# Eun0/XMC-GAN

Hardware: AMD Instinct MI355X
Metric: images/sec per G+D step (higher is better)
Workload: dtype bf16; 1 GPU; 256x256 COCO-shaped synthetic batch, 256 images per GPU, one full G+D iteration (D step + G step + Adam x2), df_gan_damsm_nomagp.yml; per_gpu_batch=256, global_batch=256, image_size=256, cfg=df_gan_damsm_nomagp.yml, parallelism=dp1, hipgraph=True, losses_finite=True, workload_name=headline

## Files before the change

### include/xmc_gan_hip.h

```cpp
#ifndef XMC_GAN_HIP_H
#define XMC_GAN_HIP_H

#include <stdint.h>

#ifdef __cplusplus
extern "C" {
#endif

#define XMC_ABI_VERSION 12

enum { XMC_BF16 = 0, XMC_F32 = 1 };
enum { XMC_HALF_IS_BF16 = 0, XMC_HALF_IS_F16 = 1 };
enum { XMC_ACT_NONE = 0, XMC_ACT_LRELU = 1, XMC_ACT_TANH = 2, XMC_ACT_RELU = 3 };
enum { XMC_EINVAL = -1, XMC_EALIGN = -2, XMC_ESHAPE = -3 };

#define XMC_MAX_TAPS 16
#define XMC_MAX_CLASSES 4

typedef struct XmcConvDesc {
    const void* src;
    const void* wpk;
    void* dst;
    const float* bias;
    const void* res;
    const float* alpha_dev;
    int32_t N, SH, SW, CS;
    int32_t DH, DW, CD;
    int32_t MH, MW;
    int32_t SA, DA;
    int32_t src_shift;
    int32_t ntaps, nclass;
    int32_t CDw;
    int32_t act;
    int32_t dtype;
    int32_t out_dtype;
    int8_t dh[XMC_MAX_CLASSES][XMC_MAX_TAPS];
    int8_t dw[XMC_MAX_CLASSES][XMC_MAX_TAPS];
    int8_t wi[XMC_MAX_CLASSES][XMC_MAX_TAPS];
    int8_t dph[XMC_MAX_CLASSES];
    int8_t dpw[XMC_MAX_CLASSES];
    const void* mask;
    float res_scale;
    int32_t res_mode;
    void* dst2;
    void* dst_pool;
    int32_t round_act;
    int32_t groups;
    int32_t post_act;
    float pool_scale;
    void* sign_bits;
    float* dot;
    const void* mask_bits;
    const void* sc_img;
    const void* sc_frag;
    const float* sc_bias;
    void* splitk_ws;
    int64_t splitk_ws_bytes;
    const void* wpk_lo;
} XmcConvDesc;

int xmc_abi_version(void);
int xmc_half_format(void);
const char* xmc_last_kernel(void);
int xmc_set_fixed_order(int on);
int xmc_set_prezeroed(int on);

int64_t xmc_conv_splitk_ws_bytes(const XmcConvDesc* d);

int xmc_conv_igemm(const XmcConvDesc* d, void* stream);

int xmc_conv_wgrad(const XmcConvDesc* d , float* dwp, void* stream);
#define XMC_BIAS_REPLICAS 16
int xmc_conv_wgrad_bias(const XmcConvDesc* d, float* dwp, float* dbias, void* stream);

int xmc_pack_weight(const float* w, void* wpk, int Co, int Ci, int KH, int KW, int rows_pad, int cols_pad,
                    int transpose , int dtype, const int32_t* row_perm , void* stream);
int xmc_pack_weight_grouped(const float* w, void* wpk, int Co, int Ci, int KH, int KW, int rows_pad, int cols_pad, int transpose,
                            int dtype, const int32_t* row_perm, int groups, void* stream);
int xmc_unpack_wgrad_grouped(const float* dwp, float* gw, int Co, int Ci, int KH, int KW, int rows_pad, int cols_pad,
                             const float* scale_dev, const int32_t* row_perm, int accumulate, int groups, void* stream);
#define XMC_PACK_MULTI_MAX 48
typedef struct XmcPackJob {
    const float* w;
    void* wpk;
    const int32_t* row_perm;
    int32_t Co, Ci, KHW, rows_pad, cols_pad, transpose, dtype, groups, upconv;
    int32_t lo;
} XmcPackJob;
int xmc_pack_weight_multi(const XmcPackJob* jobs , int njobs, void* stream);
int xmc_pack_weight_upconv(const float* w, void* wpk, int Co, int Ci, int rows_pad, int cols_pad, int transpose, int dtype,
                           void* stream);
int xmc_unpack_wgrad(const float* dwp, float* gw, int Co, int Ci, int KH, int KW, int rows_pad, int cols_pad,
                     const float* scale_dev, const int32_t* row_perm, int accumulate, void* stream);
int xmc_unpack_wgrad_bias(const float* dwp, float* gw, int Co, int Ci, int KH, int KW, int rows_pad, int cols_pad,
                          const float* scale_dev, const int32_t* row_perm, int accumulate,
                          const float* gb_replicas, float* gb, int CD, void* stream);
int xmc_unpack_wgrad_bias_dot(const float* dwp, float* gw, int Co, int Ci, int KH, int KW, int rows_pad, int cols_pad,
                              const float* scale_dev, const int32_t* row_perm, int accumulate,
                              const float* gb_replicas, float* gb, int CD, const float* bias_dot, float* dot, void* stream);

int xmc_nchw_to_nhwc8(const float* src , void* dst , int N, int C, int H, int W,
                      int dtype, void* stream);
int xmc_nhwc8_to_nchw(const void* src , float* dst , int N, int C, int H, int W,
                      int dtype, void* stream);

int xmc_lrelu(const void* x, void* y, int64_t n, float slope, int dtype, void* stream);
int xmc_lrelu_mask(const void* dy, const void* ref, void* dx, int64_t n, float slope, int dtype, void* stream);
int xmc_tanh(const void* x, void* y, int64_t n, int dtype, void* stream);
int xmc_signmask_apply(const void* dy, const void* bits, void* dx, int64_t n, float slope, int dtype, void* stream);
int xmc_conv_pw1x1_masked_src(const XmcConvDesc* d, const void* src_bits, void* src_masked, float slope, void* stream);
int xmc_conv_pw1x1_split(const XmcConvDesc* d, void* stream);
int xmc_conv_ptile_bits(const XmcConvDesc* d, void* stream);
int xmc_conv_ptile_scimg(const XmcConvDesc* d, void* stream);
int xmc_conv_wgrad_bits(const XmcConvDesc* d, float* dwp, void* stream);
int xmc_gtail_bwd(const XmcConvDesc* d, const void* img, float* dwp, float* dbias, int dw_rows, int grid_cap, void* stream);
int xmc_tanh_bwd(const void* dy, const void* y, void* dx, int64_t n, int dtype, void* stream);
int xmc_axpby(const void* a, const void* b, const float* alpha_dev, void* y, int64_t n, int dtype, void* stream);
int xmc_axpby_up(const void* a, const void* b, const float* alpha_dev, void* y, int N, int H, int W, int C, int dtype, void* stream);
int xmc_axpby_up_lrelu(const void* a, const void* b, const float* alpha_dev, void* y, int N, int H, int W, int C, int dtype, void* stream);
int xmc_scale(const void* x, const float* alpha_dev, void* y, int64_t n, int dtype, void* stream);
int xmc_dot(const void* a, const void* b, float* out, int64_t n, int dtype, void* stream);
enum { XMC_GP_BIAS = 1, XMC_GP_RELU = 2, XMC_GP_MASK = 4, XMC_GP_ATOMIC = 8 };
typedef struct XmcGemmProblem {
    const float* A;
    const float* B;
    const float* bias;
    const float* mask;
    float* C;
    float* rowsum;
    int32_t M, N, K;
    int32_t sa_i, sa_r, sb_j, sb_r;
    int32_t flags;
    int32_t tile0;
    int32_t reserved;
} XmcGemmProblem;
int xmc_gemm_group(const XmcGemmProblem* problems, int nproblems, void* stream);
int xmc_embedding_gather(const int64_t* ids, const float* table, float* out, int64_t n_tokens, int dim, int64_t vocab, void* stream);
int xmc_gru_bidir(const float* xproj, const float* w_hh, const float* b_hn, const int32_t* lens, float* words, float* sent, int B, int T,
                  int H, void* stream);
int xmc_lstm_bidir(const float* xproj, const float* w_hh, const int32_t* lens, float* words, float* sent, int B, int T, int H,
                   void* stream);
int xmc_roberta_embed_ln(const int64_t* ids, const int32_t* lens, const float* word, const float* pos, const float* type0,
                         const float* gamma, const float* beta, float* out, void* out16, int B, int T, int H, int64_t vocab, int npos,
                         int pad_idx, float eps, void* stream);
int xmc_add_layernorm(const float* x, const float* bias, const float* res, const float* gamma, const float* beta, float* out, void* out16,
                      int64_t rows, int H, float eps, void* stream);
int xmc_attention_short(const float* qkv, const int32_t* lens, void* out, int B, int T, int heads, int head_dim, int out_dtype,
                        void* stream);
int xmc_bias_gelu(const float* x, const float* bias, void* out, int64_t rows, int F, int out_dtype, void* stream);
int xmc_sbert_pool(const float* hidden, const int32_t* lens, float* words, float* sent, uint8_t* mask, int B, int T, int H, int L,
                   int normalize, void* stream);
int xmc_spectral_sigma(const float* W, float* u, float* v, float* scratch, float* sig, float* w_eff, int R, int C, int training,
                       float eps, void* stream);
int xmc_spectral_bwd(const float* g, const float* W, const float* u, const float* v, const float* sig, float* dot, float* dW,
                     int R, int C, void* stream);
int xmc_scale_mask_dot(const void* dy, const void* ref, const float* alpha_dev, void* g, float* dot, int64_t n, int dtype, void* stream);
int xmc_axpby_bwd(const void* dy, const void* b, const float* alpha_dev, void* db, void* da, float* dot,
                  int N, int H, int W, int C, int up, const void* ymask , int dtype, void* stream);
int xmc_colsum(const void* x, float* out, int64_t rows, int C, int dtype, void* stream);
int xmc_avgpool2(const void* x, void* y, int N, int H, int W, int C, int dtype, void* stream);
int xmc_upsample2(const void* x, void* y, int N, int H, int W, int C, float scale, int dtype, void* stream);
int xmc_sumpool2(const void* x, void* y, int N, int H, int W, int C, float scale, int dtype, void* stream);
int xmc_global_avgpool(const void* x, void* y, int N, int HW, int C, int dtype, int out_dtype, void* stream);
int xmc_global_avgpool_bwd(const void* dy, void* dx, int N, int HW, int C, int dtype, int in_dtype, void* stream);

int xmc_affine2_lrelu_fwd(const void* x, const float* g0, const float* b0, const float* g1, const float* b1,
                          void* y, int N, int HW, int C, int dtype, void* stream);
int xmc_affine2_lrelu_bwd(const void* x, const void* dy, const float* g0, const float* b0, const float* g1,
                          const float* b1, void* dx, float* dg0, float* db0, float* dg1, float* db1,
                          int N, int HW, int C, int dtype, void* stream);

int xmc_affine2_act_fwd(const void* x, const float* g0, const float* b0, const float* g1, const float* b1,
                        void* y, int N, int HW, int C, float slope, int dtype, void* stream);
int xmc_affine2_act_bwd(const void* x, const void* dy, const float* g0, const float* b0, const float* g1,
                        const float* b1, void* dx, float* dg0, float* db0, float* dg1, float* db1,
                        int N, int HW, int C, float slope, int dtype, void* stream);
int xmc_affine2_act_bwd_acc(const void* x, const void* dy, const float* g0, const float* b0, const float* g1,
                            const float* b1, void* dx, float* dg0, float* db0, float* dg1, float* db1, const void* dx_in,
                            int N, int HW, int C, float slope, int dtype, void* stream);
int xmc_affine2_act_bwd_dot(const void* x, const void* dy, const float* g0, const float* b0, const float* g1,
                            const float* b1, void* dx, float* dg0, float* db0, float* dg1, float* db1, const void* dx_in,
                            const float* alpha_dev, float* dot, int N, int HW, int C, float slope, int dtype, void* stream);
int xmc_affine2_act_bwd_dot_pool(const void* x, const void* dy, const float* g0, const float* b0, const float* g1,
                                 const float* b1, void* dx, float* dg0, float* db0, float* dg1, float* db1, const void* dx_in,
                                 const float* alpha_dev, float* dot, void* dx_pool, int N, int H, int W, int C, float slope,
                                 int dtype, void* stream);

int xmc_groupnorm_fwd(const void* x, const float* w, const float* b, void* y, float* stats, float* ws,
                      int N, int HW, int C, int G, float eps, float slope, int dtype, void* stream);
int xmc_groupnorm_bwd(const void* x, const void* dy, const float* w, const float* b, const float* stats, void* dx,
                      float* dw, float* db, float* ws, int N, int HW, int C, int G, float slope, int dtype, void* stream);
int64_t xmc_attn_pool_ws_floats(int N, int HW);
int xmc_attn_pool_fwd(const void* key, const float* q, const void* x, float* stats, float* ctx, float* ws, int N, int HW,
                      int ncon, int pk, int px, float scale, int dtype, void* stream);
int xmc_attn_pool_bwd(const void* key, const float* q, const void* x, const float* stats, const float* ctx, const float* dctx,
                      float* dq, void* dkey, void* dx, int N, int HW, int ncon, int pk, int px, float scale, int dtype, void* stream);
int xmc_attn_pool_bwd_acc(const void* key, const float* q, const void* x, const float* stats, const float* ctx, const float* dctx,
                          float* dq, void* dkey, void* dx, const void* dx_in, int N, int HW, int ncon, int pk, int px, float scale,
                          int dtype, void* stream);

int xmc_gvec_fwd(const float* xs, const float* xg, const float* W, const float* bias, float* y, int B, int G, int O, int Is, int Ig, void* stream);
int xmc_gvec_bwd(const float* xs, const float* xg, const float* W, const float* dy, float* dxs, float* dxg, float* dW, float* dbias,
                 int B, int G, int O, int Is, int Ig, void* stream);
int xmc_reasoner_fwd(const float* x, const float* We, const float* bn_w, const float* bn_b, float* run_mean, float* run_var, int training,
                     float momentum, float eps, float* y, float* pre, float* stat, int B, void* stream);
int xmc_reasoner_bwd(const float* x, const float* We, const float* bn_w, const float* bn_b, const float* pre, const float* stat, int batch_stats,
                     const float* dy, float* dx, float* dWe, float* dbn_w, float* dbn_b, int B, void* stream);
int xmc_word_ctx_fwd(const float* st, const float* w, const unsigned char* pad, float* ctx, float* prob, int B, int T, void* stream);
int xmc_word_ctx_bwd(const float* st, const float* w, const float* prob, const float* dctx, float* dst, float* dw, int B, int T, void* stream);
int xmc_word_keys_fwd(const float* kraw, const float* gnw, const float* gnb, float eps, float* kh, float* stat, int B, int T, void* stream);
int xmc_word_keys_bwd(const float* kraw, const float* gnw, const float* gnb, const float* stat, const float* dkh, float* dkraw, float* dgnw,
                      float* dgnb, int B, int T, void* stream);
int xmc_word_pool_fwd(const void* qmap, const float* kh, const unsigned char* pad, float* ctx, int N, int HW, int ncon, int pk, int T,
                      int dtype, void* stream);
int xmc_word_pool_bwd(const void* qmap, const float* kh, const unsigned char* pad, const float* dctx, void* dq, float* dkh, int N, int HW,
                      int ncon, int pk, int T, int dtype, void* stream);

int64_t xmc_contrastive_ws_bytes(int n, int D);
int xmc_contrastive_fwd(const float* A, const float* B, const float* labels, const float* inv_num_pos,
                        int n, int D, float* loss, void* ws, void* stream);
int xmc_contrastive_bwd(const float* A, const float* B, const float* labels, const float* inv_num_pos,
                        int n, int D, const float* dloss_dev, void* ws, float* dA, float* dB, void* stream);

int xmc_cosine_scores(const float* A, const float* B, int n, int D, float* S, void* ws, void* stream);

int xmc_hinge_fwd(const void* x, int stride, float sign, float* out, int64_t n, int dtype, void* stream);
int xmc_hinge_bwd(const void* x, int stride, float sign, const float* dloss_dev, void* dx, int64_t n, int dtype,
                  void* stream);

int xmc_cast(const void* x, void* y, int64_t n, int src_dtype, int dst_dtype, void* stream);

typedef struct XmcAdamEntry {
    float* param;
    const float* grad;
    float* m;
    float* v;
    int32_t* step;
    int64_t n;
} XmcAdamEntry;
int xmc_adam_chunk_elems(void);
int xmc_adam_step(const XmcAdamEntry* table_dev, int ntensors, const int32_t* chunks_dev, int nchunks,
                  float lr, float beta1, float beta2, float eps, float grad_scale, void* stream);
enum { XMC_ADAM_CHECK = 1, XMC_ADAM_UPDATE = 2, XMC_ADAM_RESCALE = 4 };
int xmc_adam_step_scaled(const XmcAdamEntry* table_dev, int ntensors, const int32_t* chunks_dev, int nchunks,
                         float lr, float beta1, float beta2, float eps, float* scale_dev, int32_t* flags_dev,
                         int mode, float growth, float backoff, int interval, void* stream);

typedef struct XmcEmaEntry {
    float* shadow;
    const float* param;
    int64_t n;
} XmcEmaEntry;
int xmc_ema_step(const XmcEmaEntry* table_dev, int ntensors, const int32_t* chunks_dev, int nchunks, float decay, int start,
                 int32_t* num_updates_dev, const int32_t* skip_flag_dev, int bump, void* stream);
int xmc_adam_ema_step(const XmcAdamEntry* table_dev, const XmcEmaEntry* ema_table_dev, int ntensors, const int32_t* chunks_dev,
                      int nchunks, float lr, float beta1, float beta2, float eps, float grad_scale, float decay, int start,
                      int32_t* num_updates_dev, int bump, void* stream);
int xmc_adam_ema_step_scaled(const XmcAdamEntry* table_dev, const XmcEmaEntry* ema_table_dev, int ntensors,
                             const int32_t* chunks_dev, int nchunks, float lr, float beta1, float beta2, float eps,
                             float* scale_dev, int32_t* flags_dev, int mode, float growth, float backoff, int interval,
                             float decay, int start, int32_t* num_updates_dev, int bump, void* stream);

int xmc_rows_sumsq(const float* x, float* ss, int B, int64_t cols, void* stream);
int xmc_gp_finish(const float* ss, int B, float* gp, float* coef, float inv_s2, void* stream);
int xmc_rows_scale(const float* x, const float* coef, const float* g, float* y, int B, int64_t cols, void* stream);

int xmc_concept_query_fwd(const float* sent, const float* Wq, const float* gnw, const float* gnb, float* q, float* qraw,
                          int B, int E, float eps, void* stream);
// ... 81 lines not shown
```

### xmc-gan_amd/csrc/common.h

```cpp
#pragma once
#include <hip/hip_runtime.h>
#include <stdint.h>

#include "xmc_gan_hip.h"

#ifdef XMC_H16_IS_F16
typedef _Float16 xmc_h16;
#define XMC_MFMA_16x16x32 __builtin_amdgcn_mfma_f32_16x16x32_f16
#define XMC_MFMA_32x32x16 __builtin_amdgcn_mfma_f32_32x32x16_f16
#define XMC_HALF_FORMAT 1
#else
typedef __bf16 xmc_h16;
#define XMC_MFMA_16x16x32 __builtin_amdgcn_mfma_f32_16x16x32_bf16
#define XMC_MFMA_32x32x16 __builtin_amdgcn_mfma_f32_32x32x16_bf16
#define XMC_HALF_FORMAT 0
#endif
typedef __attribute__((ext_vector_type(8))) xmc_h16 bf16x8;
typedef __attribute__((ext_vector_type(4))) xmc_h16 bf16x4;
typedef __attribute__((ext_vector_type(4))) float f32x4;
typedef __attribute__((__vector_size__(4 * sizeof(short)))) short xmc_s16x4;
typedef __attribute__((ext_vector_type(4))) uint32_t u32x4;
typedef __attribute__((ext_vector_type(2))) uint32_t u32x2;

#define XMC_LRELU 0.2f

static inline int xmc_esz(int dtype) { return dtype == XMC_BF16 ? 2 : 4; }

void xmc_note_kernel(const char* fmt, ...);
void xmc_note_generic_epi(const char* kernel, int mask);
bool xmc_debug_off(const char* token);
bool xmc_fixed_order();
hipError_t xmc_zero_acc(void* p, size_t bytes, hipStream_t st);

#define XMC_LAUNCH_CHECK()                                     \
    do {                                                       \
        hipError_t e__ = hipGetLastError();                    \
        if (e__ != hipSuccess) return -(1000 + (int)e__);      \
    } while (0)

#define XMC_MAX_DYN_LDS (160 * 1024 - 1024)
#define XMC_ALLOW_BIG_LDS(kernel)                                                                                              \
    do {                                                                                                                       \
        static bool once__ = false;                                                                                            \
        if (!once__) {                                                                                                         \
            (void)hipFuncSetAttribute(reinterpret_cast<const void*>(&kernel), hipFuncAttributeMaxDynamicSharedMemorySize,      \
                                      XMC_MAX_DYN_LDS);                                                                        \
            (void)hipGetLastError();                                                                                           \
            once__ = true;                                                                                                     \
        }                                                                                                                      \
    } while (0)

__device__ __forceinline__ bf16x4 xmc_ds_read_tr16(const void* p) {
    return __builtin_bit_cast(bf16x4, __builtin_amdgcn_ds_read_tr16_b64_v4i16((__attribute__((address_space(3))) xmc_s16x4*)(p)));
}

__device__ __forceinline__ float xmc_pin_f32(float v) {
    asm("" : "+v"(v));
    return v;
}
__device__ __forceinline__ float lrelu_f(float v) { return v > 0.f ? v : XMC_LRELU * v; }
__device__ __forceinline__ float tanh_fast(float v) {
    const float e = __builtin_amdgcn_exp2f(v * 2.8853900817779268f);
    return 1.f - 2.f * __builtin_amdgcn_rcpf(e + 1.f);
}
__device__ __forceinline__ float lrelu_slope(float ref) { return ref > 0.f ? 1.f : XMC_LRELU; }
__device__ __forceinline__ float tanh_bwd_f(float dy, float y) { return xmc_pin_f32(dy * (1.f - y * y)); }
__device__ __forceinline__ u32x4 xmc_apply_sign_bits(u32x4 v, unsigned b) {
    bf16x8 h = __builtin_bit_cast(bf16x8, v);
#pragma unroll
    for (int k = 0; k < 8; ++k) {
        const float f = (float)h[k];
        h[k] = (xmc_h16)(((b >> k) & 1u) ? f : XMC_LRELU * f);
    }
    return __builtin_bit_cast(u32x4, h);
}

template <int DT> struct Vec8;
template <> struct Vec8<XMC_BF16> {
    static constexpr int BYTES = 16;
    __device__ static __forceinline__ void load(const void* p, size_t idx8, float (&v)[8]) {
        bf16x8 t = reinterpret_cast<const bf16x8*>(p)[idx8];
#pragma unroll
        for (int i = 0; i < 8; ++i) v[i] = (float)t[i];
    }
    __device__ static __forceinline__ void store(void* p, size_t idx8, const float (&v)[8]) {
        bf16x8 t;
#pragma unroll
        for (int i = 0; i < 8; ++i) t[i] = (xmc_h16)v[i];
        reinterpret_cast<bf16x8*>(p)[idx8] = t;
    }
};
template <> struct Vec8<XMC_F32> {
    static constexpr int BYTES = 32;
    __device__ static __forceinline__ void load(const void* p, size_t idx8, float (&v)[8]) {
        const f32x4* q = reinterpret_cast<const f32x4*>(p) + idx8 * 2;
        f32x4 a = q[0], b = q[1];
#pragma unroll
        for (int i = 0; i < 4; ++i) { v[i] = a[i]; v[4 + i] = b[i]; }
    }
    __device__ static __forceinline__ void store(void* p, size_t idx8, const float (&v)[8]) {
        f32x4* q = reinterpret_cast<f32x4*>(p) + idx8 * 2;
        f32x4 a, b;
#pragma unroll
        for (int i = 0; i < 4; ++i) { a[i] = v[i]; b[i] = v[4 + i]; }
        q[0] = a; q[1] = b;
    }
};

struct XcdWalk { int first, step, end; };
__device__ __forceinline__ XcdWalk xmc_xcd_walk(int ntiles) {
    const int G = (int)gridDim.x, b = (int)blockIdx.x;
#ifdef XMC_XCD_HELPER_OFF
    return XcdWalk{b, G, ntiles};
#endif
    if ((G & 7) != 0 || G < 16) return XcdWalk{b, G, ntiles};
    const int T8 = (ntiles + 7) >> 3, base = (b & 7) * T8;
    return XcdWalk{base + (b >> 3), G >> 3, base + T8 < ntiles ? base + T8 : ntiles};
}
static inline int xmc_ab_grid(int g) {
    static const bool off = xmc_debug_off("no_xcd_map");
    return (off && g >= 16 && (g & 7) == 0) ? g - 1 : g;
}

__device__ __forceinline__ float xmc_xor1(float v) {
    return __builtin_bit_cast(float, __builtin_amdgcn_mov_dpp(__builtin_bit_cast(int, v), 0xB1, 0xF, 0xF, true));
}
__device__ __forceinline__ float xmc_xor2(float v) {
    return __builtin_bit_cast(float, __builtin_amdgcn_mov_dpp(__builtin_bit_cast(int, v), 0x4E, 0xF, 0xF, true));
}
__device__ __forceinline__ float wave_sum(float v) {
#pragma unroll
    for (int o = 32; o > 0; o >>= 1) v += __shfl_xor(v, o, 64);
    return v;
}
__device__ __forceinline__ float wave_max(float v) {
#pragma unroll
    for (int o = 32; o > 0; o >>= 1) v = fmaxf(v, __shfl_xor(v, o, 64));
    return v;
}

template <int ODT>
__device__ __forceinline__ void epilogue_tail(const XmcConvDesc& d, size_t idx8, size_t ridx8, float (&v)[8], float alpha, float* dacc = nullptr) {
    if (d.sign_bits) {
        unsigned b = 0;
#pragma unroll
        for (int k = 0; k < 8; ++k) b |= (v[k] > 0.f ? 1u : 0u) << k;
        reinterpret_cast<unsigned char*>(d.sign_bits)[idx8] = (unsigned char)b;
    }
    if (d.dst2) Vec8<ODT>::store(d.dst2, idx8, v);
    if (ODT == XMC_BF16 && (d.dst2 || d.round_act)) {
#pragma unroll
        for (int k = 0; k < 8; ++k) v[k] = (float)(xmc_h16)v[k];
    }
    float mk[8];
    if (d.mask) {
        Vec8<ODT>::load(d.mask, idx8, mk);
        if (d.dot && dacc) {
#pragma unroll
            for (int k = 0; k < 8; ++k) *dacc += v[k] * mk[k];
        }
    }
    if (d.alpha_dev) {
#pragma unroll
        for (int k = 0; k < 8; ++k) v[k] *= alpha;
    }
    if (d.mask) {
#pragma unroll
        for (int k = 0; k < 8; ++k) v[k] *= lrelu_slope(mk[k]);
    }
    if (d.res) {
        const float rs = d.res_scale == 0.f ? 1.f : d.res_scale;
        float rr[8];
        Vec8<ODT>::load(d.res, ridx8, rr);
#pragma unroll
        for (int k = 0; k < 8; ++k) v[k] += rs * rr[k];
    }
    if (d.post_act == XMC_ACT_LRELU) {
#pragma unroll
        for (int k = 0; k < 8; ++k) v[k] = lrelu_f(v[k]);
    }
    Vec8<ODT>::store(d.dst, idx8, v);
}

constexpr int kEpiBias = 1, kEpiLrelu = 2, kEpiRound = 4, kEpiDst2 = 8, kEpiAlpha = 16, kEpiMask = 32, kEpiRes = 64, kEpiPost = 128, kEpiPool = 256,
              kEpiSign = 512, kEpiDot = 1024, kEpiScImg = 2048;
constexpr int kEpiGSum = kEpiBias | kEpiRound | kEpiAlpha | kEpiRes;
constexpr int kEpiDKeep = kEpiLrelu | kEpiDst2 | kEpiAlpha | kEpiRes | kEpiPool;
constexpr int kEpiDFwd = kEpiLrelu | kEpiRound | kEpiAlpha | kEpiRes | kEpiPool;
constexpr int kEpiDLast = kEpiLrelu | kEpiDst2 | kEpiAlpha | kEpiRes;
constexpr int kEpiDLin = kEpiDst2 | kEpiAlpha | kEpiMask | kEpiRes;
constexpr int kEpiDKeepS = kEpiLrelu | kEpiRound | kEpiSign | kEpiAlpha | kEpiRes | kEpiPool;
constexpr int kEpiDLastS = kEpiLrelu | kEpiRound | kEpiSign | kEpiAlpha | kEpiRes;
constexpr int kEpiDgDot = kEpiMask | kEpiAlpha | kEpiDot;
static inline int xmc_epi_mask(const XmcConvDesc& d) {
    if ((d.act != XMC_ACT_NONE && d.act != XMC_ACT_LRELU) || d.out_dtype != XMC_BF16) return -1;
    return (d.bias ? kEpiBias : 0) | (d.act == XMC_ACT_LRELU ? kEpiLrelu : 0) | ((d.round_act && !d.dst2) ? kEpiRound : 0) | (d.dst2 ? kEpiDst2 : 0) |
           (d.alpha_dev ? kEpiAlpha : 0) | (d.mask ? kEpiMask : 0) | (d.res ? kEpiRes : 0) | (d.post_act == XMC_ACT_LRELU ? kEpiPost : 0) |
           (d.dst_pool ? kEpiPool : 0) | (d.sign_bits ? kEpiSign : 0) | (d.dot ? kEpiDot : 0) | (d.sc_img ? kEpiScImg : 0);
}

__device__ __forceinline__ size_t res_index8(const XmcConvDesc& d, size_t idx8, int n, int y, int x, int a, int b, int ch8) {
    if (d.res_mode == 0) return idx8;
    if (d.res_mode == 1) return ((size_t)(n * d.MH + a) * d.MW + b) * (d.CD >> 3) + ch8;
    return ((size_t)(n * (d.DH >> 1) + (y >> 1)) * (d.DW >> 1) + (x >> 1)) * (d.CD >> 3) + ch8;
}
```

### xmc-gan_amd/csrc/conv_thin.hip

```cpp
#include "common.h"
#include <stdlib.h>

namespace {

struct ThinCfg {
    int tiles_y, tiles_x, PW, PH, dh0, dw0;
};

template <int BN>
__global__ __launch_bounds__(256) void thin_in_kernel(const XmcConvDesc d, const ThinCfg t, int ntiles) {
    constexpr int TH = 8, TW = 32, TN = BN / 16, UPL = BN / 32, KS = 3;
    __shared__ __attribute__((aligned(16))) unsigned char patch[(TH + 4) * (TW + 4) * 16];
    const int tid = threadIdx.x, lane = tid & 63, wm = tid >> 6;
    const int fr = lane & 15, fc = lane >> 4;
    const int PW = t.PW, PH = t.PH, dh0 = t.dh0, dw0 = t.dw0;
    const u32x4* __restrict__ src16 = reinterpret_cast<const u32x4*>(d.src);
    const u32x4* __restrict__ w16 = reinterpret_cast<const u32x4*>(d.wpk);

    u32x4 wf[KS][TN];
    int toff[KS];
#pragma unroll
    for (int ks = 0; ks < KS; ++ks) {
        const int tap = ks * 4 + fc;
        const bool live = tap < d.ntaps;
// ... 393 lines not shown
#pragma unroll
            for (int u = 0; u < TN / 2; ++u) {
                if (u * 32 + fc * 8 >= d.CD) continue;
                bf16x8 o;
#pragma unroll
                for (int q = 0; q < 4; ++q) {
                    const float x0 = acc[2 * u][q] + bias8[u][q], x1 = acc[2 * u + 1][q] + bias8[u][4 + q];
                    o[q] = (xmc_h16)fmaxf(x0, x0 * slope);
                    o[4 + q] = (xmc_h16)fmaxf(x1, x1 * slope);
                }
                dst8[pix * cd8 + u * 4 + fc] = o;
            }
        }
    }
}

template <int KS, int TN>
int launch_pw(const XmcConvDesc& d, int ngroups, hipStream_t st, const unsigned char* sbits, void* smasked, float mslope) {
    int nb = (ngroups + 4 * 4 - 1) / (4 * 4);
    if (nb > 256 * 8) nb = 256 * 8;
    if (d.wpk_lo) {
        if constexpr ((KS == 2 && TN == 8) || (KS == 4 && TN == 4) || (KS == 2 && TN == 2)) {
            if (smasked) return 1;
            hipLaunchKernelGGL((pw1x1_kernel<KS, TN, false, true>), dim3(nb), dim3(256), 0, st, d, ngroups, nullptr, nullptr, 0.f);
            xmc_note_kernel("pw1x1_kernel<%d, %d, false, true>", KS, TN);
            XMC_LAUNCH_CHECK();
            return 0;
        } else {
            return 1;
        }
    }
    if (smasked) hipLaunchKernelGGL((pw1x1_kernel<KS, TN, true>), dim3(nb), dim3(256), 0, st, d, ngroups, sbits, (u32x4*)smasked, mslope);
    else hipLaunchKernelGGL((pw1x1_kernel<KS, TN, false>), dim3(nb), dim3(256), 0, st, d, ngroups, nullptr, nullptr, 0.f);
    xmc_note_kernel(smasked ? "pw1x1_kernel<%d, %d, true>" : "pw1x1_kernel<%d, %d>", KS, TN);
    XMC_LAUNCH_CHECK();
    return 0;
}

template <int KS, bool MASKED = false, bool SPLIT = false>
__global__ __launch_bounds__(512) void pw1x1w_kernel(const XmcConvDesc d, int ngroups, int ncols, const unsigned char* __restrict__ sbits,
                                                     u32x4* __restrict__ smasked, float mslope) {
    extern __shared__ __attribute__((aligned(16))) unsigned char wlds[];
    constexpr int RSTR = KS * 64 * (SPLIT ? 2 : 1) + 16;
    const int tid = threadIdx.x, lane = tid & 63, fr = lane & 15, fc = lane >> 4;
    const int cs_units = d.CS >> 3, cd8 = d.CD >> 3;
    const int c0 = blockIdx.y * ncols;
    const u32x4* __restrict__ src16 = reinterpret_cast<const u32x4*>(d.src);
    const u32x4* __restrict__ w16 = reinterpret_cast<const u32x4*>(d.wpk);
    bf16x8* __restrict__ dst8 = reinterpret_cast<bf16x8*>(d.dst);
    for (int id = tid; id < ncols * KS * 4; id += 512) {
        const int row = id / (KS * 4), ch = id - row * (KS * 4);
        const int j = row >> 4, r = row & 15;
        const int lrow = (j >> 1) * 32 + (r >> 2) * 8 + (j & 1) * 4 + (r & 3);
        *reinterpret_cast<u32x4*>(wlds + row * RSTR + ch * 16) = w16[((size_t)d.wi[0][0] * d.CDw + c0 + lrow) * cs_units + ch];
        if (SPLIT) *reinterpret_cast<u32x4*>(wlds + row * RSTR + KS * 64 + ch * 16) =
                reinterpret_cast<const u32x4*>(d.wpk_lo)[((size_t)d.wi[0][0] * d.CDw + c0 + lrow) * cs_units + ch];
    }
    __syncthreads();
    const float slope = d.act == XMC_ACT_LRELU ? XMC_LRELU : 1.f;
    const int wave_g = blockIdx.x * 8 + (tid >> 6), nwaves = gridDim.x * 8;
    constexpr int UNR = 4;
    const int nu = ncols >> 5;
    for (int g0 = wave_g * UNR; g0 < ngroups; g0 += nwaves * UNR) {
        u32x4 pf[UNR][KS];
#pragma unroll
        for (int r = 0; r < UNR; ++r) {
            const int g = g0 + r < ngroups ? g0 + r : ngroups - 1;
#pragma unroll
            for (int ks = 0; ks < KS; ++ks) pf[r][ks] = src16[(size_t)(g * 16 + fr) * cs_units + ks * 4 + fc];
        }
        if (MASKED && blockIdx.y == 0) {
#pragma unroll
            for (int r = 0; r < UNR; ++r) {
                if (g0 + r >= ngroups) break;
#pragma unroll
                for (int ks = 0; ks < KS; ++ks) {
                    const size_t idx = (size_t)((g0 + r) * 16 + fr) * cs_units + ks * 4 + fc;
                    smasked[idx] = mask_unit(pf[r][ks], sbits[idx], mslope);
                }
            }
        }
        for (int u = 0; u < nu; ++u) {
            f32x4 acc[UNR][2];
#pragma unroll
            for (int r = 0; r < UNR; ++r) acc[r][0] = acc[r][1] = f32x4{0.f, 0.f, 0.f, 0.f};
            const unsigned char* const wr = wlds + (u * 32 + fr) * RSTR + fc * 16;
#pragma unroll
            for (int ks = 0; ks < KS; ++ks) {
                const bf16x8 wa = *reinterpret_cast<const bf16x8*>(wr + ks * 64), wb = *reinterpret_cast<const bf16x8*>(wr + 16 * RSTR + ks * 64);
                if (SPLIT) {
                    const bf16x8 la = *reinterpret_cast<const bf16x8*>(wr + KS * 64 + ks * 64), lb = *reinterpret_cast<const bf16x8*>(wr + 16 * RSTR + KS * 64 + ks * 64);
#pragma unroll
                    for (int r = 0; r < UNR; ++r) {
                        acc[r][0] = XMC_MFMA_16x16x32(la, __builtin_bit_cast(bf16x8, pf[r][ks]), acc[r][0], 0, 0, 0);
                        acc[r][1] = XMC_MFMA_16x16x32(lb, __builtin_bit_cast(bf16x8, pf[r][ks]), acc[r][1], 0, 0, 0);
                    }
                }
#pragma unroll
                for (int r = 0; r < UNR; ++r) {
                    acc[r][0] = XMC_MFMA_16x16x32(wa, __builtin_bit_cast(bf16x8, pf[r][ks]), acc[r][0], 0, 0, 0);
                    acc[r][1] = XMC_MFMA_16x16x32(wb, __builtin_bit_cast(bf16x8, pf[r][ks]), acc[r][1], 0, 0, 0);
                }
            }
            const int ch = c0 + u * 32 + fc * 8;
            if (ch >= d.CD) continue;
            float b8[8];
#pragma unroll
            for (int c = 0; c < 8; ++c) b8[c] = d.bias ? d.bias[ch + c] : 0.f;
#pragma unroll
            for (int r = 0; r < UNR; ++r) {
                if (g0 + r >= ngroups) break;
                bf16x8 o;
#pragma unroll
                for (int q = 0; q < 4; ++q) {
                    const float x0 = acc[r][0][q] + b8[q], x1 = acc[r][1][q] + b8[4 + q];
                    o[q] = (xmc_h16)fmaxf(x0, x0 * slope);
                    o[4 + q] = (xmc_h16)fmaxf(x1, x1 * slope);
                }
                dst8[((size_t)(g0 + r) * 16 + fr) * cd8 + (ch >> 3)] = o;
            }
        }
    }
}

template <int KS>
int launch_pww(const XmcConvDesc& d, int ngroups, hipStream_t st, const unsigned char* sbits, void* smasked, float mslope) {
    const bool split = d.wpk_lo != nullptr;
    if (split && smasked) return 1;
    const int RSTR = KS * 64 * (split ? 2 : 1) + 16;
    int ny = 1;
    while ((size_t)(d.CDw / ny) * RSTR > XMC_MAX_DYN_LDS || d.CDw % ny != 0 || (d.CDw / ny) % 32 != 0) {
        if (++ny > d.CDw / 32) return 1;
    }
    const int ncols = d.CDw / ny;
    const size_t lds = (size_t)ncols * RSTR;
    int nb = (ngroups + 8 * 4 - 1) / (8 * 4);
    if (nb > 256 / ny) nb = 256 / ny;
    if (nb < 1) nb = 1;
    if (split) {
        XMC_ALLOW_BIG_LDS((pw1x1w_kernel<KS, false, true>));
        hipLaunchKernelGGL((pw1x1w_kernel<KS, false, true>), dim3(nb, ny), dim3(512), lds, st, d, ngroups, ncols, nullptr, nullptr, 0.f);
        xmc_note_kernel("pw1x1w_kernel<%d, false, true>", KS);
        XMC_LAUNCH_CHECK();
        return 0;
    }
    if (smasked) {
        XMC_ALLOW_BIG_LDS((pw1x1w_kernel<KS, true>));
        hipLaunchKernelGGL((pw1x1w_kernel<KS, true>), dim3(nb, ny), dim3(512), lds, st, d, ngroups, ncols, sbits, (u32x4*)smasked, mslope);
    } else {
        XMC_ALLOW_BIG_LDS((pw1x1w_kernel<KS, false>));
        hipLaunchKernelGGL((pw1x1w_kernel<KS, false>), dim3(nb, ny), dim3(512), lds, st, d, ngroups, ncols, nullptr, nullptr, 0.f);
    }
    xmc_note_kernel(smasked ? "pw1x1w_kernel<%d, true>" : "pw1x1w_kernel<%d>", KS);
    XMC_LAUNCH_CHECK();
    return 0;
}

constexpr int TO_H = 8, TO_W = 16, TO_PH = TO_H + 2, TO_PW = TO_W + 2;
template <int KC>
__global__ __launch_bounds__(256, 2) void thin_out_kernel(const XmcConvDesc d, int tiles_x, int tiles_y, int ntiles) {
    constexpr int NKS = 9 * KC, CSU = 4 * KC, PSTR = CSU * 16 + 16;
    constexpr int NUN = TO_PH * TO_PW * CSU, MAXU = (NUN + 255) / 256;
    __shared__ __attribute__((aligned(16))) unsigned char smem[TO_PH * TO_PW * PSTR];
    const int tid = threadIdx.x, lane = tid & 63, wave = tid >> 6;
    const int col = lane & 15, kb = lane >> 4;
    const u32x4* __restrict__ src = reinterpret_cast<const u32x4*>(d.src);
    const u32x4* __restrict__ wpk = reinterpret_cast<const u32x4*>(d.wpk);
    bf16x8 wa[NKS];
    int loff[9];
#pragma unroll
    for (int t = 0; t < 9; ++t) {
        loff[t] = ((d.dh[0][t] + 1) * TO_PW + d.dw[0][t] + 1 + col) * PSTR + kb * 16;
#pragma unroll
        for (int c = 0; c < KC; ++c)
            wa[t * KC + c] = __builtin_bit_cast(bf16x8, wpk[((size_t)d.wi[0][t] * d.CDw + col) * CSU + c * 4 + kb]);
    }
    float bias4[4] = {0.f, 0.f, 0.f, 0.f};
    if (d.bias && kb < 2) {
#pragma unroll
        for (int i = 0; i < 4; ++i) bias4[i] = d.bias[kb * 4 + i];
    }
    u32x4 pv[MAXU];
    auto prefetch = [&](int tile) {
        const int n = tile / (tiles_y * tiles_x), tr = tile - n * (tiles_y * tiles_x);
        const int y0 = (tr / tiles_x) * TO_H - 1, x0 = (tr % tiles_x) * TO_W - 1;
#pragma unroll
        for (int it = 0; it < MAXU; ++it) {
            const int id = tid + it * 256;
            const int pp = id / CSU, ch = id - pp * CSU;
            const int py = pp / TO_PW, px = pp - py * TO_PW;
            const int sy = y0 + py, sx = x0 + px;
            const bool ok = id < NUN && (unsigned)sy < (unsigned)d.SH && (unsigned)sx < (unsigned)d.SW;
            const u32x4 z = {0, 0, 0, 0};
            pv[it] = ok ? src[(((size_t)n * d.SH + sy) * d.SW + sx) * CSU + ch] : z;
        }
    };
    const XcdWalk xw = xmc_xcd_walk(ntiles);
    int tile = xw.first;
    if (tile < xw.end) prefetch(tile);
    for (; tile < xw.end; tile += xw.step) {
        __syncthreads();
#pragma unroll
        for (int it = 0; it < MAXU; ++it) {
            const int id = tid + it * 256;
            const int pp = id / CSU, ch = id - pp * CSU;
            if (id < NUN) *reinterpret_cast<u32x4*>(smem + pp * PSTR + ch * 16) = pv[it];
        }
        __syncthreads();
        if (tile + xw.step < xw.end) prefetch(tile + xw.step);
        const int n = tile / (tiles_y * tiles_x), tr = tile - n * (tiles_y * tiles_x);
        const int y0 = (tr / tiles_x) * TO_H, x0 = (tr % tiles_x) * TO_W;
#pragma unroll
        for (int rr = 0; rr < 2; ++rr) {
            const int r = wave * 2 + rr;
            f32x4 acc = {0.f, 0.f, 0.f, 0.f};
#pragma unroll
            for (int t = 0; t < 9; ++t)
#pragma unroll
                for (int c = 0; c < KC; ++c) {
                    const bf16x8 b = *reinterpret_cast<const bf16x8*>(smem + r * TO_PW * PSTR + loff[t] + c * 64);
                    acc = XMC_MFMA_16x16x32(wa[t * KC + c], b, acc, 0, 0, 0);
                }
            if (kb < 2) {
                bf16x4 o;
#pragma unroll
                for (int i = 0; i < 4; ++i) {
                    float v = acc[i] + bias4[i];
                    if (d.act == XMC_ACT_TANH) v = tanh_fast(v);
                    else if (d.act == XMC_ACT_LRELU) v = lrelu_f(v);
                    o[i] = (xmc_h16)v;
                }
                const size_t p = ((size_t)n * d.DH + y0 + r) * d.DW + x0 + col;
                *reinterpret_cast<bf16x4*>(reinterpret_cast<xmc_h16*>(d.dst) + p * 8 + kb * 4) = o;
            }
        }
    }
}

}

int xmc_conv_thin_out_try(const XmcConvDesc* d, void* stream) {
    static const bool off = xmc_debug_off("no_thin_out");
    if (off) return 1;
    if (d->dtype != XMC_BF16 || d->out_dtype != XMC_BF16 || d->CD != 8 || (d->CS != 32 && d->CS != 64) || d->CDw < 16) return 1;
    if (d->SA != 1 || d->DA != 1 || d->src_shift != 0 || d->nclass != 1 || d->ntaps != 9 || d->groups > 1) return 1;
    if (d->res || d->mask || d->alpha_dev || d->dst2 || d->dst_pool || d->post_act || d->sign_bits || d->dot) return 1;
    if (d->act != XMC_ACT_NONE && d->act != XMC_ACT_TANH && d->act != XMC_ACT_LRELU) return 1;
    if (d->MH % TO_H != 0 || d->MW % TO_W != 0 || d->SH != d->MH || d->SW != d->MW || d->DH != d->MH || d->DW != d->MW) return 1;
    if (d->dph[0] != 0 || d->dpw[0] != 0) return 1;
    for (int k = 0; k < 9; ++k)
        if (d->dh[0][k] < -1 || d->dh[0][k] > 1 || d->dw[0][k] < -1 || d->dw[0][k] > 1) return 1;
    const int tx = d->MW / TO_W, ty = d->MH / TO_H, ntiles = d->N * tx * ty;
    const int grid = ntiles < 256 * 8 ? ntiles : 256 * 8;
    hipStream_t st = reinterpret_cast<hipStream_t>(stream);
    if (d->CS == 32) hipLaunchKernelGGL((thin_out_kernel<1>), dim3(xmc_ab_grid(grid)), dim3(256), 0, st, *d, tx, ty, ntiles);
    else hipLaunchKernelGGL((thin_out_kernel<2>), dim3(xmc_ab_grid(grid)), dim3(256), 0, st, *d, tx, ty, ntiles);
    xmc_note_kernel("thin_out_kernel<%d>", d->CS / 32);
    XMC_LAUNCH_CHECK();
    return 0;
}

int xmc_conv_thin_try(const XmcConvDesc* d, void* stream) {
    static const bool off = xmc_debug_off("no_thin");
    if (off) return 1;
    if (d->dtype != XMC_BF16 || d->out_dtype != XMC_BF16 || d->CS != 8) return 1;
    if (d->SA != 1 || d->DA != 1 || d->src_shift != 0 || d->nclass != 1 || d->ntaps > 12) return 1;
    if (d->CDw != 32 && d->CDw != 64) return 1;
    if (d->res || d->alpha_dev || d->dst2 || d->post_act || d->sign_bits || d->dot || (d->act != XMC_ACT_NONE && d->act != XMC_ACT_LRELU)) return 1;
    if (d->MH % 8 != 0 || d->MW % 32 != 0 || d->SH != d->MH || d->SW != d->MW || d->DH != d->MH || d->DW != d->MW) return 1;
    if (d->dph[0] != 0 || d->dpw[0] != 0) return 1;
    int hmin = 127, hmax = -128, wmin = 127, wmax = -128;
    for (int k = 0; k < d->ntaps; ++k) {
        const int h = d->dh[0][k], w = d->dw[0][k];
        hmin = h < hmin ? h : hmin; hmax = h > hmax ? h : hmax;
        wmin = w < wmin ? w : wmin; wmax = w > wmax ? w : wmax;
    }
    if (hmax - hmin > 4 || wmax - wmin > 4 || hmin > 0 || wmin > 0 || hmax < 0 || wmax < 0) return 1;
    ThinCfg t;
    t.tiles_y = d->MH / 8; t.tiles_x = d->MW / 32;
    t.PH = 8 + (hmax - hmin); t.PW = 32 + (wmax - wmin);
    t.dh0 = hmin; t.dw0 = wmin;
    if (t.PH * t.PW > 512) return 1;
    const int ntiles = d->N * t.tiles_y * t.tiles_x;
    int gx = 256 * 5;
    if (gx > ntiles) gx = ntiles;
    hipStream_t st = reinterpret_cast<hipStream_t>(stream);
    if (d->CDw == 32) {
        hipLaunchKernelGGL((thin_in_kernel<32>), dim3(xmc_ab_grid(gx)), dim3(256), 0, st, *d, t, ntiles);
    } else {
        hipLaunchKernelGGL((thin_in_kernel<64>), dim3(xmc_ab_grid(gx)), dim3(256), 0, st, *d, t, ntiles);
    }
    xmc_note_kernel("thin_in_kernel<%d>", d->CDw);
    XMC_LAUNCH_CHECK();
    return 0;
}

extern "C" int xmc_gtail_bwd(const XmcConvDesc* d, const void* img, float* dwp, float* dbias, int dw_rows, int grid_cap, void* stream) {
    if (!d || !d->src || !d->wpk || !d->dst || !d->mask || !img) return XMC_EINVAL;
    if (d->N < 1 || d->MH < 1 || d->MW < 1 || d->ntaps < 1 || d->ntaps > XMC_MAX_TAPS) return XMC_ESHAPE;
    if (dwp && (dw_rows < 4 || dw_rows % 4 != 0)) return XMC_ESHAPE;
    if (d->mask_bits || d->sc_img || d->wpk_lo) return XMC_EINVAL;
    static const bool off = xmc_debug_off("no_gtail_fused");
    if (off) return 1;
    if (d->dtype != XMC_BF16 || d->out_dtype != XMC_BF16 || d->CS != 8 || d->CD != 32 || d->CDw != 32) return 1;
    if (d->SA != 1 || d->DA != 1 || d->src_shift != 0 || d->nclass != 1 || d->ntaps != 9 || d->groups > 1) return 1;
    if (d->bias || d->res || d->alpha_dev || d->dst2 || d->post_act || d->sign_bits || d->dot || d->act != XMC_ACT_NONE) return 1;
    if (d->MH % 8 != 0 || d->MW % 2 != 0 || d->SH != d->MH || d->SW != d->MW || d->DH != d->MH || d->DW != d->MW) return 1;
    if (d->dph[0] != 0 || d->dpw[0] != 0) return 1;
    for (int t = 0; t < 9; ++t)
        if (d->dh[0][t] != 1 - t / 3 || d->dw[0][t] != 1 - t % 3 || d->wi[0][t] != t) return 1;
    const int tiles_y = d->MH / 8, tiles_x = (d->MW + 31) / 32;
    if ((int64_t)d->N * d->MH * d->MW * 4 >= (1ll << 31) || (int64_t)d->N * tiles_y * tiles_x >= (1ll << 30)) return 1;
    const int ntiles = d->N * tiles_y * tiles_x;
    int gx = 256 * (dwp ? 3 : 5);
    if (grid_cap > 0 && gx > grid_cap) gx = grid_cap;
    if (gx > ntiles) gx = ntiles;
    hipStream_t st = reinterpret_cast<hipStream_t>(stream);
    const u32x4* img16 = reinterpret_cast<const u32x4*>(img);
    if (dwp) hipLaunchKernelGGL((gtail_bwd_kernel<true>), dim3(xmc_ab_grid(gx)), dim3(256), 0, st, *d, img16, dwp, dbias, dw_rows, tiles_y, tiles_x, ntiles);
    else hipLaunchKernelGGL((gtail_bwd_kernel<false>), dim3(xmc_ab_grid(gx)), dim3(256), 0, st, *d, img16, nullptr, nullptr, 0, tiles_y, tiles_x, ntiles);
    xmc_note_kernel("gtail_bwd_kernel<%d>", dwp ? 1 : 0);
    XMC_LAUNCH_CHECK();
    return 0;
}

static int pw1x1_go(const XmcConvDesc* d, void* stream, const unsigned char* sbits, void* smasked, float mslope) {
    static const bool off = xmc_debug_off("no_pw1x1");
    if (off) return 1;
    if (d->dtype != XMC_BF16 || d->out_dtype != XMC_BF16) return 1;
    if (d->ntaps != 1 || d->nclass != 1 || d->SA != 1 || d->DA != 1 || d->src_shift != 0) return 1;
    if (d->dh[0][0] != 0 || d->dw[0][0] != 0 || d->dph[0] != 0 || d->dpw[0] != 0) return 1;
    if (d->SH != d->MH || d->SW != d->MW || d->DH != d->MH || d->DW != d->MW) return 1;
    if (d->post_act || d->sign_bits || d->dot) return 1;
    if (d->res || d->mask || d->alpha_dev || d->dst2 || (d->act != XMC_ACT_NONE && d->act != XMC_ACT_LRELU)) return 1;
    if (d->CS % 32 != 0 || d->CDw % 32 != 0 || d->CD % 8 != 0) return 1;
    const int64_t M = (int64_t)d->N * d->MH * d->MW;
    if (M % 16 != 0 || M / 16 >= (1ll << 31) || M < 16 * 1024) return 1;
    const int ngroups = (int)(M / 16);
    hipStream_t st = reinterpret_cast<hipStream_t>(stream);
    const int ks = d->CS / 32, tn = d->CDw / 16;
    static const bool no_w = xmc_debug_off("no_pw1x1_lds");
    if (!no_w && (ks == 4 || ks == 8) && ks * tn > 16 && d->CDw >= 128 && M >= 32 * 1024)
        return ks == 4 ? launch_pww<4>(*d, ngroups, st, sbits, smasked, mslope) : launch_pww<8>(*d, ngroups, st, sbits, smasked, mslope);
    if (d->CS > 128 || d->CDw > 128) return 1;
    if (ks * tn > 16 || ks == 3) return 1;
#define PW_CASE(K, T) if (ks == K && tn == T) return launch_pw<K, T>(*d, ngroups, st, sbits, smasked, mslope);
    PW_CASE(1, 2) PW_CASE(1, 4) PW_CASE(1, 8) PW_CASE(2, 2) PW_CASE(2, 4) PW_CASE(2, 8) PW_CASE(4, 2) PW_CASE(4, 4)
#undef PW_CASE
    return 1;
}

int xmc_conv_pw1x1_try(const XmcConvDesc* d, void* stream) { return d->wpk_lo ? 1 : pw1x1_go(d, stream, nullptr, nullptr, 0.f); }

extern "C" int xmc_conv_pw1x1_split(const XmcConvDesc* d, void* stream) {
    if (!d || !d->src || !d->wpk || !d->wpk_lo || !d->dst) return XMC_EINVAL;
    if (d->ntaps != 1 || d->CS % 8 != 0 || d->CD % 8 != 0 || d->CDw % 32 != 0 || d->CDw < d->CD || d->N < 1 || d->MH < 1 || d->MW < 1) return XMC_ESHAPE;
    if (d->mask_bits || d->sc_img) return XMC_EINVAL;
    static const bool off = xmc_debug_off("no_pw1x1_split");
    if (off) return 1;
    return pw1x1_go(d, stream, nullptr, nullptr, 0.f);
}

extern "C" int xmc_conv_pw1x1_masked_src(const XmcConvDesc* d, const void* src_bits, void* src_masked, float slope, void* stream) {
    if (!d || !d->src || !d->wpk || !d->dst || !src_bits || !src_masked) return XMC_EINVAL;
    if (d->ntaps != 1 || d->CS % 8 != 0 || d->CD % 8 != 0 || d->CDw % 32 != 0 || d->CDw < d->CD || d->N < 1 || d->MH < 1 || d->MW < 1) return XMC_ESHAPE;
    static const bool off = xmc_debug_off("no_pw1x1_masked_src");
    if (off) return 1;
    return pw1x1_go(d, stream, static_cast<const unsigned char*>(src_bits), src_masked, slope);
}
```

### xmc-gan_amd/csrc/pointwise.hip

```cpp
#include "common.h"
#include <stdlib.h>
#include <string.h>
#include <cstdarg>
#include <cstdio>

namespace {

constexpr int NT = 256;
inline int nblocks(int64_t items, int per_block = NT, int cap = 256 * 16) {
    int64_t b = (items + per_block - 1) / per_block;
    if (b < 1) b = 1;
    return (int)(b > cap ? cap : b);
}

constexpr int UN = 4;
constexpr int STREAM_BLOCKS = 1024;
inline int sblocks(int64_t n8) { return nblocks((n8 + UN - 1) / UN, NT, STREAM_BLOCKS); }

template <int DT, class F>
__global__ void map1_kernel(const void* x, void* y, int64_t n8, F f) {
    for (int64_t base = (int64_t)blockIdx.x * (NT * UN); base < n8; base += (int64_t)gridDim.x * (NT * UN)) {
        float v[UN][8];
#pragma unroll
        for (int j = 0; j < UN; ++j) {
// ... 175 lines not shown
    }
    __shared__ float red[NT * 8];
#pragma unroll
    for (int k = 0; k < 8; ++k) red[threadIdx.x * 8 + k] = s[k];
    __syncthreads();
    if (threadIdx.x < c8_here) {
        float t[8] = {0, 0, 0, 0, 0, 0, 0, 0};
        for (int gg = 0; gg < groups; ++gg)
#pragma unroll
            for (int k = 0; k < 8; ++k) t[k] += red[(gg * c8_here + threadIdx.x) * 8 + k];
#pragma unroll
        for (int k = 0; k < 8; ++k) atomicAdd(&out[(c8_base + threadIdx.x) * 8 + k], t[k]);
    }
}

template <int DT>
__global__ void pool2_kernel(const void* x, void* y, int N, int H, int W, int C8, float scale) {
    const int OH = H / 2, OW = W / 2;
    const int64_t total = (int64_t)N * OH * OW * C8;
    for (int64_t i = blockIdx.x * (int64_t)blockDim.x + threadIdx.x; i < total; i += (int64_t)gridDim.x * blockDim.x) {
        int cc = (int)(i % C8);
        int64_t p = i / C8;
        int ow = (int)(p % OW); p /= OW;
        int oh = (int)(p % OH);
        int n = (int)(p / OH);
        float acc[8] = {0, 0, 0, 0, 0, 0, 0, 0}, v[8];
#pragma unroll
        for (int dy = 0; dy < 2; ++dy)
#pragma unroll
            for (int dx = 0; dx < 2; ++dx) {
                Vec8<DT>::load(x, (((int64_t)n * H + 2 * oh + dy) * W + 2 * ow + dx) * C8 + cc, v);
#pragma unroll
                for (int k = 0; k < 8; ++k) acc[k] += v[k];
            }
#pragma unroll
        for (int k = 0; k < 8; ++k) acc[k] *= scale;
        Vec8<DT>::store(y, i, acc);
    }
}
template <int DT>
__global__ void up2_kernel(const void* x, void* y, int N, int H, int W, int C8, float scale) {
    const int OH = H * 2, OW = W * 2;
    const int64_t total = (int64_t)N * OH * OW * C8;
    for (int64_t i = blockIdx.x * (int64_t)blockDim.x + threadIdx.x; i < total; i += (int64_t)gridDim.x * blockDim.x) {
        int cc = (int)(i % C8);
        int64_t p = i / C8;
        int ow = (int)(p % OW); p /= OW;
        int oh = (int)(p % OH);
        int n = (int)(p / OH);
        float v[8];
        Vec8<DT>::load(x, (((int64_t)n * H + (oh >> 1)) * W + (ow >> 1)) * C8 + cc, v);
#pragma unroll
        for (int k = 0; k < 8; ++k) v[k] *= scale;
        Vec8<DT>::store(y, i, v);
    }
}
template <int DT, int OD>
__global__ void gap_kernel(const void* x, void* y, int N, int HW, int C8) {
    const int64_t total = (int64_t)N * C8;
    for (int64_t i = blockIdx.x * (int64_t)blockDim.x + threadIdx.x; i < total; i += (int64_t)gridDim.x * blockDim.x) {
        int cc = (int)(i % C8);
        int n = (int)(i / C8);
        float acc[8] = {0, 0, 0, 0, 0, 0, 0, 0}, v[8];
        for (int p = 0; p < HW; ++p) {
            Vec8<DT>::load(x, ((int64_t)n * HW + p) * C8 + cc, v);
#pragma unroll
            for (int k = 0; k < 8; ++k) acc[k] += v[k];
        }
        const float inv = 1.f / HW;
#pragma unroll
        for (int k = 0; k < 8; ++k) acc[k] *= inv;
        Vec8<OD>::store(y, i, acc);
    }
}
template <int DT>
__global__ void gap_big_kernel(const void* x, float* y, int HW, int C8, int pix_per_block) {
    const int n = blockIdx.y, groups = NT / C8;
    const int cc = threadIdx.x % C8, g = threadIdx.x / C8;
    float acc[8] = {0, 0, 0, 0, 0, 0, 0, 0}, v[8];
    const int p_end = min(HW, (int)(blockIdx.x + 1) * pix_per_block);
    if (g < groups)
        for (int p = blockIdx.x * pix_per_block + g; p < p_end; p += groups) {
            Vec8<DT>::load(x, ((size_t)n * HW + p) * C8 + cc, v);
#pragma unroll
            for (int k = 0; k < 8; ++k) acc[k] += v[k];
        }
    __shared__ float red[NT * 8];
#pragma unroll
    for (int k = 0; k < 8; ++k) red[threadIdx.x * 8 + k] = acc[k];
    __syncthreads();
    if (threadIdx.x < C8) {
        const float inv = 1.f / HW;
        float t[8] = {0, 0, 0, 0, 0, 0, 0, 0};
        for (int gg = 0; gg < groups; ++gg)
#pragma unroll
            for (int k = 0; k < 8; ++k) t[k] += red[(gg * C8 + threadIdx.x) * 8 + k];
#pragma unroll
        for (int k = 0; k < 8; ++k) atomicAdd(&y[((size_t)n * C8 + threadIdx.x) * 8 + k], t[k] * inv);
    }
}
template <int DT, int ID>
__global__ void gap_bwd_kernel(const void* dy, void* dx, int N, int HW, int C8) {
    const int64_t total = (int64_t)N * HW * C8;
    const float inv = 1.f / HW;
    for (int64_t i = blockIdx.x * (int64_t)blockDim.x + threadIdx.x; i < total; i += (int64_t)gridDim.x * blockDim.x) {
        int cc = (int)(i % C8);
        int n = (int)(i / ((int64_t)HW * C8));
        float v[8];
        Vec8<ID>::load(dy, (int64_t)n * C8 + cc, v);
#pragma unroll
        for (int k = 0; k < 8; ++k) v[k] *= inv;
        Vec8<DT>::store(dx, i, v);
    }
}

template <int DT>
__global__ void nchw_to_nhwc8_kernel(const float* src, void* dst, int N, int C, int HW) {
    const int64_t total = (int64_t)N * HW;
    for (int64_t i = blockIdx.x * (int64_t)blockDim.x + threadIdx.x; i < total; i += (int64_t)gridDim.x * blockDim.x) {
        int64_t n = i / HW, p = i - n * HW;
        float v[8] = {0, 0, 0, 0, 0, 0, 0, 0};
        for (int c = 0; c < C; ++c) v[c] = src[(n * C + c) * HW + p];
        Vec8<DT>::store(dst, i, v);
    }
}
template <int DT>
__global__ void nhwc8_to_nchw_kernel(const void* src, float* dst, int N, int C, int HW) {
    const int64_t total = (int64_t)N * HW;
    for (int64_t i = blockIdx.x * (int64_t)blockDim.x + threadIdx.x; i < total; i += (int64_t)gridDim.x * blockDim.x) {
        int64_t n = i / HW, p = i - n * HW;
        float v[8];
        Vec8<DT>::load(src, i, v);
        for (int c = 0; c < C; ++c) dst[(n * C + c) * HW + p] = v[c];
    }
}

template <int DT>
__global__ void affine2_fwd_kernel(const void* x, const float* g0, const float* b0, const float* g1, const float* b1,
                                   void* y, int HW, int C8, int pix_per_block, float slope) {
    const int n = blockIdx.y, groups = NT / C8;
    const int cc = threadIdx.x % C8, g = threadIdx.x / C8;
    if (g >= groups) return;
    float G0[8], B0[8], G1[8], B1[8];
    const size_t pb = ((size_t)n * C8 + cc) * 8;
    const bool two = g1 != nullptr;
#pragma unroll
    for (int k = 0; k < 8; ++k) { G0[k] = g0[pb + k]; B0[k] = b0[pb + k]; G1[k] = two ? g1[pb + k] : 1.f; B1[k] = two ? b1[pb + k] : 0.f; }
    const int p_end = min(HW, (int)(blockIdx.x + 1) * pix_per_block);
    for (int p = blockIdx.x * pix_per_block + g; p < p_end; p += groups) {
        float v[8];
        const size_t idx = ((size_t)n * HW + p) * C8 + cc;
        Vec8<DT>::load(x, idx, v);
#pragma unroll
        for (int k = 0; k < 8; ++k) {
            float u = v[k] * G0[k] + B0[k];
            u = u > 0.f ? u : slope * u;
            const float t = u * G1[k] + B1[k];
            v[k] = two ? (t > 0.f ? t : slope * t) : u;
        }
        Vec8<DT>::store(y, idx, v);
    }
}
template <int DT, bool POOL>
__global__ __launch_bounds__(NT, 2) void affine2_bwd_kernel(
                                   const void* x, const void* dy, const float* g0, const float* b0, const float* g1,
                                   const float* b1, void* dx, float* dg0, float* db0, float* dg1, float* db1,
                                   int HW, int C8, int pix_per_block, float slope, const void* dx_in,
                                   const float* alpha_dev, float* dot, void* dx_pool, int Wq) {
    const float al = alpha_dev ? *alpha_dev : 1.f;
    float dacc = 0.f;
    const int n = blockIdx.y, groups = NT / C8;
    const int cc = threadIdx.x % C8, g = threadIdx.x / C8;
    float G0[8], B0[8], G1[8], B1[8];
    float sg0[8], sb0[8], sg1[8], sb1[8];
    const size_t pb = ((size_t)n * C8 + cc) * 8;
    const bool two = g1 != nullptr;
#pragma unroll
    for (int k = 0; k < 8; ++k) {
        G0[k] = g0[pb + k]; B0[k] = b0[pb + k]; G1[k] = two ? g1[pb + k] : 1.f; B1[k] = two ? b1[pb + k] : 0.f;
        sg0[k] = sb0[k] = sg1[k] = sb1[k] = 0.f;
    }
    auto pixel = [&](size_t idx, float (&xv)[8], const float (&dv)[8], const float (&o)[8], float* acc8) {
#pragma unroll
        for (int k = 0; k < 8; ++k) {
            float u = xv[k] * G0[k] + B0[k];
            float a1 = u > 0.f ? u : slope * u;
            float v = a1 * G1[k] + B1[k];
            if (dot) {
                const float y2 = two ? (v > 0.f ? v : slope * v) : a1;
                dacc += dv[k] * (DT == XMC_BF16 ? (float)(xmc_h16)y2 : y2);
            }
            const float dvk = dv[k] * al;
            float dvv = two ? dvk * (v > 0.f ? 1.f : slope) : dvk;
            sg1[k] += dvv * a1; sb1[k] += dvv;
            float du = dvv * G1[k] * (u > 0.f ? 1.f : slope);
            sg0[k] += du * xv[k]; sb0[k] += du;
            xv[k] = du * G0[k];
        }
        if (dx_in) {
#pragma unroll
            for (int k = 0; k < 8; ++k) xv[k] += o[k];
        }
        Vec8<DT>::store(dx, idx, xv);
        if (POOL) {
#pragma unroll
            for (int k = 0; k < 8; ++k) acc8[k] += DT == XMC_BF16 ? (float)(xmc_h16)xv[k] : xv[k];
        }
    };
    const int p_end = min(HW, (int)(blockIdx.x + 1) * pix_per_block);
    if (g < groups)
        for (int p = blockIdx.x * pix_per_block + g; p < p_end; p += POOL ? groups : 2 * groups) {
            if (!POOL) {
                float xv[8], dv[8], o[8], xw[8], dw[8], ow[8];
                const size_t idx = ((size_t)n * HW + p) * C8 + cc;
                const bool second = p + groups < p_end;
                const size_t idx2 = second ? idx + (size_t)groups * C8 : idx;
                Vec8<DT>::load(x, idx, xv);
                Vec8<DT>::load(x, idx2, xw);
                Vec8<DT>::load(dy, idx, dv);
                Vec8<DT>::load(dy, idx2, dw);
                if (dx_in) { Vec8<DT>::load(dx_in, idx, o); Vec8<DT>::load(dx_in, idx2, ow); }
                pixel(idx, xv, dv, o, nullptr);
                if (second) pixel(idx2, xw, dw, ow, nullptr);
            } else {
                const int W = 2 * Wq;
                const int qy = p / W, col = p - qy * W;
                const size_t i0 = (((size_t)n * (HW / W) * 2 + 2 * qy) * W + col) * C8 + cc, i1 = i0 + (size_t)W * C8;
                float x0[8], d0[8], o0[8], x1[8], d1[8], o1[8];
                Vec8<DT>::load(x, i0, x0); Vec8<DT>::load(x, i1, x1);
                Vec8<DT>::load(dy, i0, d0); Vec8<DT>::load(dy, i1, d1);
                if (dx_in) { Vec8<DT>::load(dx_in, i0, o0); Vec8<DT>::load(dx_in, i1, o1); }
                float acc8[8] = {0, 0, 0, 0, 0, 0, 0, 0};
                pixel(i0, x0, d0, o0, acc8);
                pixel(i1, x1, d1, o1, acc8);
#pragma unroll
                for (int k = 0; k < 8; ++k) acc8[k] += __shfl_xor(acc8[k], C8, 64);
                if ((col & 1) == 0) Vec8<DT>::store(dx_pool, (((size_t)n * (HW / W) + qy) * Wq + (col >> 1)) * C8 + cc, acc8);
            }
        }
    if (dot) {
        dacc = wave_sum(dacc);
        if ((threadIdx.x & 63) == 0) atomicAdd(dot, dacc);
    }
    __shared__ float red[NT * 8];
    float* outs[4] = {dg0, db0, dg1, db1};
    float* sums[4] = {sg0, sb0, sg1, sb1};
#pragma unroll
    for (int q = 0; q < 4; ++q) {
        if (!two && q >= 2) break;
        __syncthreads();
#pragma unroll
        for (int k = 0; k < 8; ++k) red[threadIdx.x * 8 + k] = sums[q][k];
        __syncthreads();
        if (threadIdx.x < C8) {
            float t[8] = {0, 0, 0, 0, 0, 0, 0, 0};
            for (int gg = 0; gg < groups; ++gg)
#pragma unroll
                for (int k = 0; k < 8; ++k) t[k] += red[(gg * C8 + threadIdx.x) * 8 + k];
#pragma unroll
            for (int k = 0; k < 8; ++k) atomicAdd(&outs[q][((size_t)n * C8 + threadIdx.x) * 8 + k], t[k]);
        }
    }
}

template <int DT>
__global__ void hinge_fwd_kernel(const void* x, int stride, float sign, float* out, int64_t n) {
    float s = 0.f;
    for (int64_t i = threadIdx.x; i < n; i += blockDim.x) {
        float v = DT == XMC_BF16 ? (float)reinterpret_cast<const xmc_h16*>(x)[i * stride] : reinterpret_cast<const float*>(x)[i * stride];
        s += fmaxf(1.f + sign * v, 0.f);
    }
    s = wave_sum(s);
    __shared__ float part[NT / 64];
    if ((threadIdx.x & 63) == 0) part[threadIdx.x >> 6] = s;
    __syncthreads();
    if (threadIdx.x == 0) {
        float t = 0.f;
        for (int w = 0; w < NT / 64; ++w) t += part[w];
        *out = t / (float)n;
    }
}
template <int DT>
__global__ void hinge_bwd_kernel(const void* x, int stride, float sign, const float* dloss, void* dx, int64_t n) {
    const float gscale = (*dloss) * sign / (float)n;
    for (int64_t i = blockIdx.x * (int64_t)blockDim.x + threadIdx.x; i < n; i += (int64_t)gridDim.x * blockDim.x) {
        float v = DT == XMC_BF16 ? (float)reinterpret_cast<const xmc_h16*>(x)[i * stride] : reinterpret_cast<const float*>(x)[i * stride];
        float gval = (1.f + sign * v) > 0.f ? gscale : 0.f;
        if (DT == XMC_BF16) reinterpret_cast<xmc_h16*>(dx)[i * stride] = (xmc_h16)gval;
        else reinterpret_cast<float*>(dx)[i * stride] = gval;
    }
}

__device__ __forceinline__ float pack_value(const float* __restrict__ w, int Co, int Ci, int KHW, int rows_pad, int cols_pad,
                                            int transpose, const int32_t* __restrict__ row_perm, int groups, int64_t i) {
    const int cog = Co / groups, cig = Ci / groups;
    int c = (int)(i % cols_pad);
    int64_t q = i / cols_pad;
    int r = (int)(q % rows_pad);
    int t = (int)(q / rows_pad);
    int co = transpose ? c : r, ci = transpose ? r : c;
    float v = 0.f;
    if (co < Co && ci < Ci) {
        int sco = row_perm ? row_perm[co] : co;
        if (groups == 1) v = w[((int64_t)sco * Ci + ci) * KHW + t];
        else if (sco / cog == ci / cig) v = w[((int64_t)sco * cig + ci % cig) * KHW + t];
    }
    return v;
}
__device__ __forceinline__ float pack_upconv_value(const float* __restrict__ w, int Co, int Ci, int rows_pad, int cols_pad,
                                                   int transpose, int64_t idx) {
    int c = (int)(idx % cols_pad);
    int64_t q = idx / cols_pad;
    int r = (int)(q % rows_pad);
    int sl = (int)(q / rows_pad);
    int cls = sl >> 2, t = sl & 3;
    int i = cls >> 1, j = cls & 1, th = t >> 1, tw = t & 1;
    int co = transpose ? c : r, ci = transpose ? r : c;
    float v = 0.f;
    if (co < Co && ci < Ci) {
        int kh0 = (i == 0) ? (th == 0 ? 0 : 1) : (th == 0 ? 0 : 2), kh1 = (i == 0) ? (th == 0 ? 0 : 2) : (th == 0 ? 1 : 2);
        int kw0 = (j == 0) ? (tw == 0 ? 0 : 1) : (tw == 0 ? 0 : 2), kw1 = (j == 0) ? (tw == 0 ? 0 : 2) : (tw == 0 ? 1 : 2);
        const float* wp = w + ((int64_t)co * Ci + ci) * 9;
        for (int kh = kh0; kh <= kh1; ++kh)
            for (int kw = kw0; kw <= kw1; ++kw) v += wp[kh * 3 + kw];
    }
    return v;
}
template <int DT>
__global__ void pack_weight_kernel(const float* w, void* wpk, int Co, int Ci, int KHW, int rows_pad, int cols_pad,
                                   int transpose, const int32_t* row_perm, int groups) {
    const int64_t total = (int64_t)KHW * rows_pad * cols_pad;
    for (int64_t i = blockIdx.x * (int64_t)blockDim.x + threadIdx.x; i < total; i += (int64_t)gridDim.x * blockDim.x) {
        const float v = pack_value(w, Co, Ci, KHW, rows_pad, cols_pad, transpose, row_perm, groups, i);
        if (DT == XMC_BF16) reinterpret_cast<xmc_h16*>(wpk)[i] = (xmc_h16)v;
        else reinterpret_cast<float*>(wpk)[i] = v;
    }
}
template <int DT>
__global__ void pack_upconv_kernel(const float* w, void* wpk, int Co, int Ci, int rows_pad, int cols_pad, int transpose) {
    const int64_t total = (int64_t)16 * rows_pad * cols_pad;
    for (int64_t idx = blockIdx.x * (int64_t)blockDim.x + threadIdx.x; idx < total; idx += (int64_t)gridDim.x * blockDim.x) {
        const float v = pack_upconv_value(w, Co, Ci, rows_pad, cols_pad, transpose, idx);
        if (DT == XMC_BF16) reinterpret_cast<xmc_h16*>(wpk)[idx] = (xmc_h16)v;
        else reinterpret_cast<float*>(wpk)[idx] = v;
    }
}
constexpr int PM_CHUNK = 2048;
struct PackJobs { XmcPackJob j[XMC_PACK_MULTI_MAX]; int32_t first[XMC_PACK_MULTI_MAX + 1]; int32_t njobs; };
template <int DT>
__device__ __forceinline__ void pack_store(void* p, int64_t i, float v, bool lo = false) {
    if (DT == XMC_BF16) reinterpret_cast<xmc_h16*>(p)[i] = lo ? (xmc_h16)(v - (float)(xmc_h16)v) : (xmc_h16)v;
    else reinterpret_cast<float*>(p)[i] = v;
}
template <int DT>
__device__ __forceinline__ void pack_position(const XmcPackJob& job, int pos) {
// ... 622 lines not shown
```

### xmc-gan_amd/lib.py

```python
import ctypes as C
import os

HERE = os.path.dirname(os.path.abspath(__file__))
LIB_PATH = os.environ.get("XMC_LIB_PATH", os.path.join(HERE, "libxmc_gan_hip.so"))
LIB_PATH_F16 = os.environ.get("XMC_LIB_PATH_F16", os.path.join(HERE, "libxmc_gan_hip_f16.so"))
ABI_VERSION = 12

BF16, F32 = 0, 1
H16 = BF16
ACT_NONE, ACT_LRELU, ACT_TANH, ACT_RELU = 0, 1, 2, 3
MAX_TAPS, MAX_CLASSES = 16, 4
POOL_MAX, POOL_AVG_VALID, POOL_AVG_PAD = 0, 1, 2
DIFFAUG_PARTS = 64

vp, i32, i64, f32 = C.c_void_p, C.c_int32, C.c_int64, C.c_float


class ConvDesc(C.Structure):
    _fields_ = [("src", vp), ("wpk", vp), ("dst", vp), ("bias", vp), ("res", vp), ("alpha_dev", vp),
                ("N", i32), ("SH", i32), ("SW", i32), ("CS", i32),
                ("DH", i32), ("DW", i32), ("CD", i32),
                ("MH", i32), ("MW", i32), ("SA", i32), ("DA", i32), ("src_shift", i32),
                ("ntaps", i32), ("nclass", i32), ("CDw", i32), ("act", i32), ("dtype", i32), ("out_dtype", i32),
                ("dh", (C.c_int8 * MAX_TAPS) * MAX_CLASSES), ("dw", (C.c_int8 * MAX_TAPS) * MAX_CLASSES),
                ("wi", (C.c_int8 * MAX_TAPS) * MAX_CLASSES),
                ("dph", C.c_int8 * MAX_CLASSES), ("dpw", C.c_int8 * MAX_CLASSES),
                ("mask", vp), ("res_scale", f32), ("res_mode", i32), ("dst2", vp), ("dst_pool", vp), ("round_act", i32), ("groups", i32),
                ("post_act", i32), ("pool_scale", f32), ("sign_bits", vp), ("dot", vp), ("mask_bits", vp), ("sc_img", vp), ("sc_frag", vp), ("sc_bias", vp),
                ("splitk_ws", vp), ("splitk_ws_bytes", C.c_int64), ("wpk_lo", vp)]


GEMM_PROBLEM = [("A", "u8"), ("B", "u8"), ("bias", "u8"), ("mask", "u8"), ("C", "u8"), ("rowsum", "u8"),
                ("M", "i4"), ("N", "i4"), ("K", "i4"), ("sa_i", "i4"), ("sa_r", "i4"), ("sb_j", "i4"), ("sb_r", "i4"),
                ("flags", "i4"), ("tile0", "i4"), ("reserved", "i4")]
GP_BIAS, GP_RELU, GP_MASK, GP_ATOMIC = 1, 2, 4, 8


class PackJob(C.Structure):
    _fields_ = [("w", vp), ("wpk", vp), ("row_perm", vp), ("Co", i32), ("Ci", i32), ("KHW", i32), ("rows_pad", i32),
                ("cols_pad", i32), ("transpose", i32), ("dtype", i32), ("groups", i32), ("upconv", i32), ("lo", i32)]


class AdamEntry(C.Structure):
    _fields_ = [("param", vp), ("grad", vp), ("m", vp), ("v", vp), ("step", vp), ("n", i64)]


class EmaEntry(C.Structure):
    _fields_ = [("shadow", vp), ("param", vp), ("n", i64)]


_SIGS = {
    "xmc_abi_version": [],
    "xmc_half_format": [],
    "xmc_last_kernel": [],
    "xmc_set_fixed_order": [i32],
    "xmc_set_prezeroed": [i32],
    "xmc_conv_splitk_ws_bytes": [vp],
    "xmc_conv_igemm": [C.POINTER(ConvDesc), vp],
    "xmc_conv_wgrad": [C.POINTER(ConvDesc), vp, vp],
    "xmc_conv_wgrad_bias": [C.POINTER(ConvDesc), vp, vp, vp],
    "xmc_pack_weight": [vp, vp, i32, i32, i32, i32, i32, i32, i32, i32, vp, vp],
    "xmc_pack_weight_grouped": [vp, vp, i32, i32, i32, i32, i32, i32, i32, i32, vp, i32, vp],
    "xmc_pack_weight_upconv": [vp, vp, i32, i32, i32, i32, i32, i32, vp],
    "xmc_pack_weight_multi": [C.POINTER(PackJob), i32, vp],
    "xmc_axpby_up": [vp, vp, vp, vp, i32, i32, i32, i32, i32, vp],
    "xmc_unpack_wgrad": [vp, vp, i32, i32, i32, i32, i32, i32, vp, vp, i32, vp],
    "xmc_unpack_wgrad_grouped": [vp, vp, i32, i32, i32, i32, i32, i32, vp, vp, i32, i32, vp],
    "xmc_unpack_wgrad_bias": [vp, vp, i32, i32, i32, i32, i32, i32, vp, vp, i32, vp, vp, i32, vp],
    "xmc_unpack_wgrad_bias_dot": [vp, vp, i32, i32, i32, i32, i32, i32, vp, vp, i32, vp, vp, i32, vp, vp, vp],
    "xmc_nchw_to_nhwc8": [vp, vp, i32, i32, i32, i32, i32, vp],
    "xmc_nhwc8_to_nchw": [vp, vp, i32, i32, i32, i32, i32, vp],
    "xmc_lrelu": [vp, vp, i64, f32, i32, vp],
    "xmc_lrelu_mask": [vp, vp, vp, i64, f32, i32, vp],
    "xmc_tanh": [vp, vp, i64, i32, vp],
    "xmc_signmask_apply": [vp, vp, vp, i64, f32, i32, vp],
    "xmc_conv_pw1x1_masked_src": [C.POINTER(ConvDesc), vp, vp, f32, vp],
    "xmc_conv_pw1x1_split": [C.POINTER(ConvDesc), vp],
    "xmc_conv_ptile_bits": [C.POINTER(ConvDesc), vp],
    "xmc_conv_ptile_scimg": [C.POINTER(ConvDesc), vp],
    "xmc_conv_wgrad_bits": [C.POINTER(ConvDesc), vp, vp],
    "xmc_gtail_bwd": [C.POINTER(ConvDesc), vp, vp, vp, i32, i32, vp],
    "xmc_tanh_bwd": [vp, vp, vp, i64, i32, vp],
    "xmc_axpby": [vp, vp, vp, vp, i64, i32, vp],
    "xmc_scale_mask_dot": [vp, vp, vp, vp, vp, i64, i32, vp],
    "xmc_axpby_bwd": [vp, vp, vp, vp, vp, vp, i32, i32, i32, i32, i32, vp, i32, vp],
    "xmc_axpby_up_lrelu": [vp, vp, vp, vp, i32, i32, i32, i32, i32, vp],
    "xmc_scale": [vp, vp, vp, i64, i32, vp],
    "xmc_dot": [vp, vp, vp, i64, i32, vp],
    "xmc_gemm_group": [vp, i32, vp],
    "xmc_embedding_gather": [vp, vp, vp, i64, i32, i64, vp],
    "xmc_lstm_bidir": [vp, vp, vp, vp, vp, i32, i32, i32, vp],
    "xmc_gru_bidir": [vp, vp, vp, vp, vp, vp, i32, i32, i32, vp],
    "xmc_roberta_embed_ln": [vp, vp, vp, vp, vp, vp, vp, vp, vp, i32, i32, i32, i64, i32, i32, f32, vp],
    "xmc_add_layernorm": [vp, vp, vp, vp, vp, vp, vp, i64, i32, f32, vp],
    "xmc_attention_short": [vp, vp, vp, i32, i32, i32, i32, i32, vp],
    "xmc_bias_gelu": [vp, vp, vp, i64, i32, i32, vp],
    "xmc_sbert_pool": [vp, vp, vp, vp, vp, i32, i32, i32, i32, i32, vp],
    "xmc_spectral_sigma": [vp, vp, vp, vp, vp, vp, i32, i32, i32, f32, vp],
    "xmc_spectral_bwd": [vp, vp, vp, vp, vp, vp, vp, i32, i32, vp],
    "xmc_colsum": [vp, vp, i64, i32, i32, vp],
    "xmc_avgpool2": [vp, vp, i32, i32, i32, i32, i32, vp],
    "xmc_upsample2": [vp, vp, i32, i32, i32, i32, f32, i32, vp],
    "xmc_sumpool2": [vp, vp, i32, i32, i32, i32, f32, i32, vp],
    "xmc_global_avgpool": [vp, vp, i32, i32, i32, i32, i32, vp],
    "xmc_global_avgpool_bwd": [vp, vp, i32, i32, i32, i32, i32, vp],
    "xmc_affine2_act_fwd": [vp, vp, vp, vp, vp, vp, i32, i32, i32, f32, i32, vp],
    "xmc_affine2_act_bwd": [vp, vp, vp, vp, vp, vp, vp, vp, vp, vp, vp, i32, i32, i32, f32, i32, vp],
    "xmc_affine2_act_bwd_acc": [vp, vp, vp, vp, vp, vp, vp, vp, vp, vp, vp, vp, i32, i32, i32, f32, i32, vp],
    "xmc_affine2_act_bwd_dot": [vp, vp, vp, vp, vp, vp, vp, vp, vp, vp, vp, vp, vp, vp, i32, i32, i32, f32, i32, vp],
    "xmc_affine2_act_bwd_dot_pool": [vp, vp, vp, vp, vp, vp, vp, vp, vp, vp, vp, vp, vp, vp, vp, i32, i32, i32, i32, f32, i32, vp],
    "xmc_affine2_lrelu_fwd": [vp, vp, vp, vp, vp, vp, i32, i32, i32, i32, vp],
    "xmc_affine2_lrelu_bwd": [vp, vp, vp, vp, vp, vp, vp, vp, vp, vp, vp, i32, i32, i32, i32, vp],
    "xmc_groupnorm_fwd": [vp, vp, vp, vp, vp, vp, i32, i32, i32, i32, f32, f32, i32, vp],
    "xmc_groupnorm_bwd": [vp, vp, vp, vp, vp, vp, vp, vp, vp, i32, i32, i32, i32, f32, i32, vp],
    "xmc_attn_pool_ws_floats": [i32, i32],
    "xmc_attn_pool_fwd": [vp, vp, vp, vp, vp, vp, i32, i32, i32, i32, i32, f32, i32, vp],
    "xmc_attn_pool_bwd": [vp, vp, vp, vp, vp, vp, vp, vp, vp, i32, i32, i32, i32, i32, f32, i32, vp],
    "xmc_attn_pool_bwd_acc": [vp, vp, vp, vp, vp, vp, vp, vp, vp, vp, i32, i32, i32, i32, i32, f32, i32, vp],
    "xmc_word_pool_fwd": [vp, vp, vp, vp, i32, i32, i32, i32, i32, i32, vp],
    "xmc_word_pool_bwd": [vp, vp, vp, vp, vp, vp, i32, i32, i32, i32, i32, i32, vp],
    "xmc_gvec_fwd": [vp, vp, vp, vp, vp, i32, i32, i32, i32, i32, vp],
    "xmc_gvec_bwd": [vp, vp, vp, vp, vp, vp, vp, vp, i32, i32, i32, i32, i32, vp],
    "xmc_reasoner_fwd": [vp, vp, vp, vp, vp, vp, i32, f32, f32, vp, vp, vp, i32, vp],
    "xmc_reasoner_bwd": [vp, vp, vp, vp, vp, vp, i32, vp, vp, vp, vp, vp, i32, vp],
    "xmc_word_ctx_fwd": [vp, vp, vp, vp, vp, i32, i32, vp],
    "xmc_word_ctx_bwd": [vp, vp, vp, vp, vp, vp, i32, i32, vp],
    "xmc_word_keys_fwd": [vp, vp, vp, f32, vp, vp, i32, i32, vp],
    "xmc_word_keys_bwd": [vp, vp, vp, vp, vp, vp, vp, vp, i32, i32, vp],
    "xmc_contrastive_ws_bytes": [i32, i32],
    "xmc_contrastive_fwd": [vp, vp, vp, vp, i32, i32, vp, vp, vp],
    "xmc_contrastive_bwd": [vp, vp, vp, vp, i32, i32, vp, vp, vp, vp, vp],
    "xmc_cosine_scores": [vp, vp, i32, i32, vp, vp, vp],
    "xmc_hinge_fwd": [vp, i32, f32, vp, i64, i32, vp],
    "xmc_hinge_bwd": [vp, i32, f32, vp, vp, i64, i32, vp],
    "xmc_cast": [vp, vp, i64, i32, i32, vp],
    "xmc_concept_query_fwd": [vp, vp, vp, vp, vp, vp, i32, i32, f32, vp],
    "xmc_concept_query_bwd": [vp, vp, vp, vp, vp, vp, vp, vp, vp, vp, i32, i32, f32, vp],
    "xmc_concept_query_fwd_multi": [vp, vp, vp, vp, i32, vp, vp, i32, i32, f32, vp],
    "xmc_concept_query_bwd_multi": [vp, vp, vp, i32, vp, vp, vp, vp, vp, vp, i32, i32, f32, vp],
    "xmc_concept_gquery_fwd": [vp, vp, vp, vp, vp, vp, i32, f32, vp],
    "xmc_concept_gquery_bwd": [vp, vp, vp, vp, vp, vp, vp, vp, vp, i32, f32, vp],
    "xmc_concept_head_fwd": [vp, vp, vp, vp, vp, vp, i32, i32, vp],
    "xmc_concept_head_fwd_pre": [vp, vp, vp, vp, vp, vp, vp, i32, i32, vp],
    "xmc_concept_head_bwd_pre": [vp, vp, vp, vp, vp, vp, vp, vp, vp, vp, i32, i32, vp],
    "xmc_concept_outer_multi": [vp, vp, vp, vp, i32, i32, vp, i32, i32, i32, vp],
    "xmc_concept_head_bwd": [vp, vp, vp, vp, vp, vp, vp, vp, vp, vp, i32, i32, vp],
    "xmc_rows_sumsq": [vp, vp, i32, i64, vp],
    "xmc_gp_finish": [vp, i32, vp, vp, f32, vp],
    "xmc_rows_scale": [vp, vp, vp, vp, i32, i64, vp],
    "xmc_adam_chunk_elems": [],
    "xmc_adam_step": [vp, i32, vp, i32, f32, f32, f32, f32, f32, vp],
    "xmc_adam_step_scaled": [vp, i32, vp, i32, f32, f32, f32, f32, vp, vp, i32, f32, f32, i32, vp],
    "xmc_ema_step": [vp, i32, vp, i32, f32, i32, vp, vp, i32, vp],
    "xmc_adam_ema_step": [vp, vp, i32, vp, i32, f32, f32, f32, f32, f32, f32, i32, vp, i32, vp],
    "xmc_adam_ema_step_scaled": [vp, vp, i32, vp, i32, f32, f32, f32, f32, vp, vp, i32, f32, f32, i32, f32, i32, vp, i32, vp],
    "xmc_dstem_compose": [vp, vp, vp, vp, vp, vp, vp, vp, vp, vp],
    "xmc_dstem_compose_bwd": [vp, vp, vp, vp, vp, vp, vp, vp, vp, vp, vp, vp, vp, vp],
    "xmc_dstem_pack": [vp, vp, vp],
    "xmc_dstem_pack_sc": [vp, vp, vp],
    "xmc_dstem_fwd": [vp, vp, vp, vp, vp, i32, i32, i32, f32, vp],
    "xmc_dstem_wgrad": [vp, vp, vp, vp, vp, i32, i32, i32, i32, vp],
    "xmc_dstem_border_fwd": [vp, vp, vp, vp, vp, vp, vp, i32, i32, i32, f32, vp],
    "xmc_dstem_border_wgrad": [vp, vp, vp, vp, i32, i32, i32, vp],
    "xmc_dstem_dgrad": [vp, vp, vp, vp, vp, vp, i32, i32, i32, vp],
    "xmc_diffaug_sums": [vp, vp, vp, i32, i32, i32, i32, i32, i32, i32, vp],
    "xmc_diffaug_apply": [vp, vp, vp, vp, i32, i32, i32, i32, i32, i32, i32, i32, vp],
    "xmc_image_to_u8": [vp, vp, i32, i32, i32, i32, vp],
    "xmc_image_minmax": [vp, vp, i32, i32, i32, i32, vp],
    "xmc_image_grid_u8": [vp, vp, vp, i32, i32, i32, i32, i32, i32, vp],
    "xmc_fid_resize_u8": [vp, vp, i32, i32, i32, i32, i32, vp],
    "xmc_pool3x3": [vp, vp, i32, i32, i32, i32, i32, i32, vp],
    "xmc_fid_moments": [vp, vp, vp, i32, i32, vp],
    "xmc_resize_bilinear_f32": [vp, vp, i32, i32, i32, i32, i32, vp],
    "xmc_rprecision": [vp, vp, vp, vp, vp, i32, i32, i32, i32, vp],
    "xmc_crop_flip_normalize": [vp, i64, vp, vp, i32, vp, vp, vp, i32, i32, vp],
    "xmc_caption_gather": [vp, vp, i64, vp, vp, i32, vp, i32, i32, i32, vp, vp, vp, vp],
    "xmc_manifold_slices": [i32, i32, i32],
    "xmc_row_sqnorm": [vp, vp, i32, i32, vp],
    "xmc_knn_radius2": [vp, vp, vp, vp, i64, i32, i32, i32, i32, vp],
    "xmc_manifold_count": [vp, vp, vp, vp, vp, vp, vp, vp, i64, i32, i32, i32, i32, vp],
    "xmc_poly_mmd_tiles": [i32],
    "xmc_poly_mmd_sums": [vp, vp, vp, vp, vp, vp, i64, i32, i32, i32, i32, i32, vp],
    "xmc_inception_score_ws_bytes": [i32, i32, i32],
    "xmc_inception_score": [vp, i64, vp, vp, vp, i64, i32, i32, i32, vp],
}
_RESTYPE = {"xmc_contrastive_ws_bytes": i64, "xmc_conv_splitk_ws_bytes": i64, "xmc_attn_pool_ws_floats": i64, "xmc_last_kernel": C.c_char_p,
            "xmc_inception_score_ws_bytes": i64}
EXPORTS = tuple(_SIGS)

_libs = {}
_variant = "bf16"


class XmcHipError(RuntimeError):
    pass


def use_variant(v):
    global _variant
    assert v in ("bf16", "f16")
    _variant = v


def variant():
    return _variant


def load(v=None):
    v = v or _variant
    lib = _libs.get(v)
    if lib is not None:
        return lib
    path = LIB_PATH if v == "bf16" else LIB_PATH_F16
    if not os.path.exists(path):
        raise RuntimeError(
            f"{path} is missing: build it with `make -C xmc-gan_amd/csrc` (or __graft_entry__.build()). "
            "The XMC-GAN step has no CPU/PyTorch fallback.")
    lib = C.CDLL(path)
    for name, args in _SIGS.items():
        fn = getattr(lib, name)
        fn.argtypes = args
        fn.restype = _RESTYPE.get(name, C.c_int)
    if lib.xmc_abi_version() != ABI_VERSION:
        raise RuntimeError(f"{path}: ABI version {lib.xmc_abi_version()}, this binding needs {ABI_VERSION} (stale build?)")
    if lib.xmc_half_format() != (0 if v == "bf16" else 1):
        raise RuntimeError(f"{path} was not built for the {v} storage format")
    lib.xmc_set_prezeroed(1)
    _libs[v] = lib
    return lib


_ECODES = {-1: "XMC_EINVAL (bad argument)", -2: "XMC_EALIGN (alignment / channel multiple)", -3: "XMC_ESHAPE (shape out of range)"}


# ... 10 lines not shown
```

### xmc-gan_amd/ops/_engine.py

```python
import ctypes as C
import weakref
import torch
from .. import lib as L
from .. import prof
from ._config import (
    _DEBUG_DISPATCH, _code, _nbytes, _need_cuda, _p, _st, _weights_epoch, bump_weights_epoch, chan_pad, pad_to)


class ConvGeom:

    __slots__ = ("cin", "cout", "k", "s", "p", "row_perm", "_perm_dev", "groups", "kh", "kw", "ph", "pw")

    def __init__(self, cin, cout, k=1, s=1, p=0, row_perm=None, groups=1):
        self.kh, self.kw = k if isinstance(k, (tuple, list)) else (k, k)
        self.ph, self.pw = p if isinstance(p, (tuple, list)) else (p, p)
        assert self.kh >= 1 and self.kw >= 1 and self.kh * self.kw <= 127 and s >= 1
        assert cin % groups == 0 and cout % groups == 0
        self.cin, self.cout, self.s = cin, cout, s
        self.k = self.kh if self.kh == self.kw else None
        self.p = self.ph if self.ph == self.pw else None
        self.groups = groups
        self.row_perm = row_perm
        self._perm_dev = None

# ... 508 lines not shown
    if isinstance(shape, int):
        shape = (shape,)
    if "no_arena_scalars" in _DEBUG_DISPATCH:
        return torch.zeros(tuple(shape), dtype=torch.float32, device=device)
    return _escape.zeros(tuple(shape), torch.device(device))


def new_iteration(device):
    _arena.new_iteration(torch.device(device))
    _escape.new_iteration(torch.device(device))
    _pooled_grads.clear()


def end_iteration(device):
    _arena.end_iteration(torch.device(device))


_pooled_grads = {}


def _pool_key(t):
    return (t.data_ptr(), tuple(t.shape), t.dtype)


def _pooled_put(dx, dxp):
    _pooled_grads[_pool_key(dx)] = (dx, dx._version, dxp)


def _pooled_take(dz):
    ent = _pooled_grads.pop(_pool_key(dz), None)
    if ent is None:
        return None
    dx, ver, dxp = ent
    same = dx.untyped_storage().data_ptr() == dz.untyped_storage().data_ptr() and dx.stride() == dz.stride() and dx._version == ver
    return dxp if same else None


def _conv_wgrad_raw(x, dy, geom, scale=None, up=False, want_bias=False, bias_dot=None, dot=None):
    staged = dy if isinstance(dy, _StagedMask) else None
    if staged is not None:
        dy = staged.dy
    _need_cuda(x, dy)
    N, H, W, CS = x.shape
    _, OH, OW, CDy = dy.shape
    assert x.dtype == dy.dtype, (x.dtype, dy.dtype)
    rows = pad_to(CDy, 32)
    dwp = _arena.zeros((geom.k * geom.k, rows, CS), x.device)
    gb = _arena.zeros((16, CDy), x.device) if want_bias else None
    d = L.ConvDesc()
    d.src, d.dst = x.data_ptr(), dy.data_ptr()
    d.N, d.SH, d.SW, d.CS = N, H, W, CS
    d.DH, d.DW, d.CD = OH, OW, CDy
    d.MH, d.MW, d.SA, d.DA, d.src_shift = OH, OW, geom.s, 1, 1 if up else 0
    d.ntaps, d.nclass, d.CDw = geom.k * geom.k, 1, rows
    d.dtype, d.out_dtype = _code(x.dtype), L.F32
    d.groups = geom.groups
    _fill_taps(d, 0, [(kh - geom.p, kw - geom.p, kh * geom.k + kw) for kh in range(geom.k) for kw in range(geom.k)])
    rc = 1
    if staged is not None and not want_bias:
        d.mask_bits = staged.bits.data_ptr()
        with prof.launch("wgrad_kernel (conv weight gradient, MFMA + split-K atomics)", 2.0 * N * OH * OW * geom.cout * geom.cin * geom.k * geom.k,
                         f"wgrad+bits {x.dtype} N{N} {H}x{W} {geom.cin}->{geom.cout} k{geom.k}s{geom.s}", _nbytes(x, dy, dwp)):
            rc = L.load().xmc_conv_wgrad_bits(C.byref(d), _p(dwp), _st())
        if rc not in (0, 1):
            L.check(rc, "xmc_conv_wgrad_bits")
        d.mask_bits = None
    if rc == 1:
        if staged is not None:
            d.dst = staged.materialised().data_ptr()
        with prof.launch("wgrad_kernel (conv weight gradient, MFMA + split-K atomics)", 2.0 * N * OH * OW * geom.cout * geom.cin * geom.k * geom.k,
                         f"wgrad {x.dtype} N{N} {H}x{W} {geom.cin}->{geom.cout} k{geom.k}s{geom.s}", _nbytes(x, dy, dwp)):
            L.check(L.load().xmc_conv_wgrad_bias(C.byref(d), _p(dwp), _p(gb), _st()), "xmc_conv_wgrad")
    return _wgrad_unpack(dwp, gb, geom, rows, CS, CDy, scale, bias_dot, dot)


def _wgrad_unpack(dwp, gb, geom, rows, CS, CDy, scale=None, bias_dot=None, dot=None):
    gw = torch.empty((geom.cout, geom.cin // geom.groups, geom.k, geom.k), dtype=torch.float32, device=dwp.device)
    if gb is not None:
        assert geom.groups == 1
        gbs = torch.empty(CDy, dtype=torch.float32, device=dwp.device)
        assert (bias_dot is None) == (dot is None)
        L.call("xmc_unpack_wgrad_bias_dot", _p(dwp), _p(gw), geom.cout, geom.cin, geom.k, geom.k, rows, CS, _p(scale),
               _p(geom.perm_dev(dwp.device)), 0, _p(gb), _p(gbs), CDy, _p(bias_dot), _p(dot), _st())
        return gw, gbs
    assert bias_dot is None
    L.call("xmc_unpack_wgrad_grouped", _p(dwp), _p(gw), geom.cout, geom.cin, geom.k, geom.k, rows, CS, _p(scale),
           _p(geom.perm_dev(dwp.device)), 0, geom.groups, _st())
    return gw


def _gtail_bwd_raw(dy, img, y, w, geom, want_w, want_bias, grid_cap=0):
    N, H, W, CS = y.shape
    if (_code(y.dtype) != L.BF16 or CS != 32 or geom.cout > 4 or geom.k != 3 or geom.s != 1 or geom.p != 1 or geom.groups != 1
            or H % 8 or W % 2 or "no_gtail_fused" in _DEBUG_DISPATCH):
        return None
    _need_cuda(dy, img, y, w)
    assert dy.shape == img.shape == (N, H, W, 8) and dy.dtype == img.dtype == y.dtype and img.is_contiguous() and y.is_contiguous()
    d, dz, dsc, _wpk = _dgrad_desc(dy, w, geom, (H, W), y.dtype, mask=y, want_sumpool=True)
    rows = pad_to(8, 32)
    dwp = _arena.zeros((9, rows, CS), y.device) if want_w else None
    gb = _arena.zeros((16, 8), y.device) if want_w and want_bias else None
    with prof.launch("gtail_bwd_kernel (conv_out dgrad + wgrad + tanh', one pass)", 2.0 * N * H * W * 8 * 32 * 9 * (2 if want_w else 1),
                     f"gtail-bwd {y.dtype} N{N} {H}x{W} {geom.cin}->{geom.cout}", _nbytes(dy, img, y, dz, dsc)):
        rc = L.load().xmc_gtail_bwd(C.byref(d), _p(img), _p(dwp), _p(gb), rows, int(grid_cap), _st())
    if rc == 1:
        return None
    L.check(rc, "xmc_gtail_bwd")
    if not want_w:
        return dz, dsc, None, None
    r = _wgrad_unpack(dwp, gb, geom, rows, CS, 8)
    gw, gbs = r if gb is not None else (r, None)
    return dz, dsc, gw, gbs


def _axpby_bwd_fused(dy, b, alpha, up, ymask=None, want_db=True):
    dy = dy.contiguous()
    N, OH, OW, Cc = dy.shape
    H, W = (OH // 2, OW // 2) if up else (OH, OW)
    al = alpha.detach().reshape(-1).float()
    db = torch.empty_like(dy) if want_db else None
    da = torch.empty((N, H, W, Cc), dtype=dy.dtype, device=dy.device) if (up or ymask is not None) else None
    dot = _zeros_f32_out(1, dy.device)
    L.call("xmc_axpby_bwd", _p(dy), _p(b), _p(al), _p(db), _p(da), _p(dot), N, H, W, Cc, 1 if up else 0, _p(ymask), _code(dy.dtype), _st())
    return da, db, dot.reshape(alpha.shape).to(alpha.dtype)


def _affine_fwd_raw(x, ps, slope):
    N, H, W, Cc = x.shape
    for t in ps:
        assert t.shape == (N, Cc), (t.shape, (N, Cc))
    y = torch.empty_like(x)
    ptrs = [_p(t) for t in ps] + ([] if len(ps) == 4 else [None, None])
    L.call("xmc_affine2_act_fwd", _p(x), *ptrs, _p(y), N, H * W, Cc, float(slope), _code(x.dtype), _st())
    return y


def _affine_bwd_raw(x, dy, ps, slope, dx_acc=None, alpha=None, dot=None, want_sumpool=False):
    N, H, W, Cc = x.shape
    dx = torch.empty_like(x)
    if dx_acc is not None:
        dx_acc = dx_acc.contiguous()
        assert dx_acc.shape == x.shape and dx_acc.dtype == x.dtype
    nred = len(ps)
    red = _zeros_f32((nred, N, Cc), x.device)
    ptrs = [_p(t) for t in ps] + ([] if nred == 4 else [None, None])
    rptrs = [_p(red[i]) for i in range(nred)] + ([] if nred == 4 else [None, None])
    assert (alpha is None) == (dot is None)
    dxp = torch.empty((N, H // 2, W // 2, Cc), dtype=x.dtype, device=x.device) if want_sumpool else None
    L.call("xmc_affine2_act_bwd_dot_pool", _p(x), _p(dy), *ptrs, _p(dx), *rptrs, _p(dx_acc), _p(alpha), _p(dot), _p(dxp), N, H, W, Cc,
           float(slope), _code(x.dtype), _st())
    return (dx, red, dxp) if want_sumpool else (dx, red)


def compose_dstem(w_img, b_img, w0, ws, bs):
    F = torch.nn.functional
    co, mid = w0.shape[0], w0.shape[1]
    w0, b_img = w0.float(), b_img.float()
    wie = F.pad(w_img.float(), (0, 0, 0, 0, 0, 8 - w_img.shape[1]))
    wa = F.conv_transpose2d(w0, wie)
    box = torch.full((1, 1, 2, 2), 0.25, dtype=torch.float32, device=w_img.device)
    wp = F.conv_transpose2d(wie.reshape(mid * 8, 1, 3, 3), box).reshape(mid, 8, 4, 4)
    wb = torch.einsum("om,mcab->ocab", ws.float()[:, :, 0, 0], wp)
    w = torch.cat((wa, F.pad(wb, (1, 1, 1, 1)))).permute(0, 2, 3, 1).reshape(2 * co, 36, 8)
    ba = torch.einsum("omhw,m->o", w0, b_img)
    bb = ws.float()[:, :, 0, 0] @ b_img + (bs.float() if bs is not None else 0.0)
    ct1 = F.conv_transpose1d
    lines = [-ct1(w0[:, :, 0, :], wie[:, :, 2, :]), -ct1(w0[:, :, 3, :], wie[:, :, 0, :]),
             -ct1(w0[:, :, :, 0], wie[:, :, :, 2]), -ct1(w0[:, :, :, 3], wie[:, :, :, 0])]
    corners = [(0, 0, 2, 2), (0, 3, 2, 0), (3, 0, 0, 2), (3, 3, 0, 0)]
    D = torch.cat([t.permute(0, 2, 1) for t in lines] + [(w0[:, :, kh, kw] @ wie[:, :, ih, iw]).unsqueeze(1) for kh, kw, ih, iw in corners], 1)
    DB = torch.stack([-(w0[:, :, 0, :].sum(2) @ b_img), -(w0[:, :, 3, :].sum(2) @ b_img), -(w0[:, :, :, 0].sum(2) @ b_img),
                      -(w0[:, :, :, 3].sum(2) @ b_img)] + [w0[:, :, kh, kw] @ b_img for kh, kw, _, _ in corners], 1)
    return w.contiguous(), torch.cat((ba, bb)).contiguous(), D.contiguous(), DB.contiguous()


def _dstem_compose_raw(w_img, b_img, w0, ws, bs):
    _need_cuda(w_img, w0)
    dev = w_img.device
    assert tuple(w_img.shape) == (32, 3, 3, 3) and tuple(w0.shape) == (64, 32, 4, 4) and tuple(ws.shape[:2]) == (64, 32)
    flat = torch.empty(128 * 36 * 8 + 128 + 64 * 28 * 8 + 64 * 8, dtype=torch.float32, device=dev)
    W, b = flat[:36864].view(128, 36, 8), flat[36864:36992]
    D, DB = flat[36992:36992 + 14336].view(64, 28, 8), flat[36992 + 14336:].view(64, 8)
    f = lambda t: None if t is None else t.detach().float().contiguous()
    wi_, bi_, w0_, ws_, bs_ = f(w_img), f(b_img), f(w0), f(ws), f(bs)
    L.call("xmc_dstem_compose", _p(wi_), _p(bi_), _p(w0_), _p(ws_), _p(bs_), _p(W), _p(b), _p(D), _p(DB), _st())
    return W, b, D, DB


def _dstem_compose_bwd_raw(w_img, b_img, w0, ws, bs, dW, dbias, dD, dDB):
    f = lambda t: t.detach().float().contiguous()
    wi_, bi_, w0_, ws_ = f(w_img), f(b_img), f(w0), f(ws)
    dwi, dbi, dw0, dws = (torch.empty_like(t) for t in (wi_, bi_, w0_, ws_))
    dbs = torch.empty(64, dtype=torch.float32, device=wi_.device) if bs is not None else None
    L.call("xmc_dstem_compose_bwd", _p(wi_), _p(bi_), _p(w0_), _p(ws_), _p(dW.contiguous()), _p(dbias.contiguous()), _p(dD.contiguous()),
           _p(dDB.contiguous()), _p(dwi), _p(dbi), _p(dw0), _p(dws), _p(dbs), _st())
    return dwi, dbi, dw0, dws, dbs


def _dstem_fwd_raw(xin, wsets, bias, slope=0.2, want_sc=True):
    _need_cuda(xin, wsets)
    N, H, W, _ = xin.shape
    wfrag = torch.empty(8 * 5 * 64 * 8, dtype=xin.dtype, device=xin.device)
    L.call("xmc_dstem_pack", _p(wsets), _p(wfrag), _st())
    h1 = torch.empty((N, H // 2, W // 2, 64), dtype=xin.dtype, device=xin.device)
    sc = torch.empty_like(h1) if want_sc else None
    with prof.launch("igemm_kernel (conv fwd+dgrad, MFMA implicit GEMM)", 2.0 * N * (H // 2) * (W // 2) * 64 * (3 * 36 + (3 * 16 if want_sc else 0)),
                     f"dstem-fwd {xin.dtype} N{N} {H}x{W} 3->64{'+64' if want_sc else ''} k6s2", _nbytes(xin, h1, sc)):
        L.call("xmc_dstem_fwd", _p(xin), _p(wfrag), _p(bias), _p(h1), _p(sc), N, H, W, float(slope), _st())
    return h1, sc


def _dstem_sc_operands(xin, wsets, bias):
    frag = torch.empty(4 * 2 * 64 * 8, dtype=xin.dtype, device=xin.device)
    L.call("xmc_dstem_pack_sc", _p(wsets), _p(frag), _st())
    return xin, frag, bias[64:128]


def _dstem_border_fwd_raw(xin, wsets, bias, D, DB, h1, slope=0.2):
    N, H, W, _ = xin.shape
    wt = torch.empty(64 * 1024, dtype=torch.uint8, device=xin.device)
    L.call("xmc_dstem_border_fwd", _p(xin), _p(wsets), _p(bias), _p(D), _p(DB), _p(wt), _p(h1), N, H, W, float(slope), _st())


def _dstem_dgrad_raw(dh1, dsc, wsets, D, H, W):
    _need_cuda(dh1, dsc)
    N = dh1.shape[0]
    dh1, dsc = dh1.contiguous(), dsc.contiguous()
    frag = torch.empty(36 * 1024, dtype=torch.uint8, device=dh1.device)
    dimg = torch.empty((N, H, W, 8), dtype=dh1.dtype, device=dh1.device)
    with prof.launch("igemm_kernel (conv fwd+dgrad, MFMA implicit GEMM)", 2.0 * N * (H // 2) * (W // 2) * 64 * (3 * 36 + 3 * 16),
                     f"dstem-dgrad {dh1.dtype} N{N} {H}x{W} 64+64->3 k6s2", _nbytes(dh1, dsc, dimg)):
        L.call("xmc_dstem_dgrad", _p(dh1), _p(dsc), _p(wsets), _p(D), _p(frag), _p(dimg), N, H, W, _st())
    return dimg


def _dstem_wgrad_raw(xin, dh1, dsc, skip_border=False, border=True):
    _need_cuda(xin, dh1, dsc)
    N, H, W, _ = xin.shape
    dh1, dsc = dh1.contiguous(), dsc.contiguous()
    n_w, n_d = 128 * 36 * 8, 64 * 28 * 8
    flat = _arena.zeros((n_w + 128 + n_d + 64 * 8,), xin.device)
    dw, db = flat[:n_w].view(128, 36, 8), flat[n_w:n_w + 128]
    dD, dDB = flat[n_w + 128:n_w + 128 + n_d].view(64, 28, 8), flat[n_w + 128 + n_d:].view(64, 8)
    with prof.launch("wgrad_kernel (conv weight gradient, MFMA + split-K atomics)", 2.0 * N * (H // 2) * (W // 2) * 64 * (3 * 36 + 3 * 16),
                     f"dstem-wgrad {xin.dtype} N{N} {H}x{W} 3->64+64 k6s2", _nbytes(xin, dh1, dsc)):
        L.call("xmc_dstem_wgrad", _p(xin), _p(dh1), _p(dsc), _p(dw), _p(db), N, H, W, 1 if skip_border else 0, _st())
    if border:
        L.call("xmc_dstem_border_wgrad", _p(xin), _p(dh1), _p(dD), _p(dDB), N, H, W, _st())
    return dw, db, dD, dDB
```

### xmc-gan_amd/ops/_nodes_block.py

```python
import torch
from .. import lib as L
from ._config import _DEBUG_DISPATCH, _code, _need_cuda, _p, _second_order, _skip_wgrad, _st, precise_trunk
from ._engine import (
    _StagedMask, _affine_bwd_raw, _affine_fwd_raw, _conv1x1_pair_raw, _conv_dgrad_raw, _conv_fwd_raw, _conv_wgrad_raw,
    _dstem_border_fwd_raw, _dstem_compose_bwd_raw, _dstem_compose_raw, _dstem_dgrad_raw, _dstem_fwd_raw, _dstem_sc_operands,
    _dstem_wgrad_raw, _pooled_put, _zeros_f32, _zeros_f32_out)
from ._nodes_leaf import CastFn
from ._nodes_conv import _bias_padded


class ResDFn(torch.autograd.Function):

    @staticmethod
    def forward(ctx, x, w0, w2, ws, bs, gamma, g0, g2, gs, xp_hint=None, want_pool=False):
        x = x.contiguous()
        dt = x.dtype
        N, H, W, _ = x.shape
        xp32 = None
        if xp_hint is not None and xp_hint.dtype == torch.float32 and dt != torch.float32:
            xp32 = xp_hint
            xp = None
        elif xp_hint is not None:
            xp = xp_hint
        else:
            xp = torch.empty((N, H // 2, W // 2, x.shape[3]), dtype=dt, device=x.device)
            L.call("xmc_sumpool2", _p(x), _p(xp), N, H, W, x.shape[3], 0.25, _code(dt), _st())
        bp = _bias_padded(bs, gs) if ws is not None else None
        al = gamma.detach().reshape(-1).float()
        if precise_trunk() and dt != torch.float32 and H // 2 <= 8 and not _second_order():
            if xp32 is None:
                xp32 = CastFn.apply(xp, torch.float32)
            if xp is None and ws is not None:
                xp = CastFn.apply(xp32, dt)
            sc32 = _conv_fwd_raw(xp32, ws, bp, gs, L.ACT_NONE, torch.float32) if ws is not None else xp32
            h1 = _conv_fwd_raw(x, w0, None, g0, L.ACT_LRELU, dt)
            keep = any(ctx.needs_input_grad[:6])
            r = _conv_fwd_raw(h1, w2, None, g2, L.ACT_LRELU, torch.float32, res=sc32, alpha=al, want_sign=keep)
            out32, bits = r if keep else (r, None)
            ctx.geoms, ctx.learned, ctx.has_bs = (g0, g2, gs), ws is not None, bs is not None
            ctx.save_for_backward(x, xp if ws is not None else None, h1, bits, w0, w2, ws, gamma)
            if not want_pool:
                return out32
            outp = torch.empty((N, out32.shape[1] // 2, out32.shape[2] // 2, out32.shape[3]), dtype=torch.float32, device=x.device)
            L.call("xmc_sumpool2", _p(out32), _p(outp), N, out32.shape[1], out32.shape[2], out32.shape[3], 0.25, L.F32, _st())
            out = CastFn.apply(out32, dt)
            ctx.mark_non_differentiable(outp)
            ctx.set_materialize_grads(False)
            return out, outp
        if xp is None:
            xp = CastFn.apply(xp32, dt)
        if ws is not None:
            sc = _conv1x1_pair_raw(xp, ws, bp, gs, dt) if (precise_trunk() and dt != torch.float32 and not _second_order()) else None
            if sc is None:
                sc = _conv_fwd_raw(xp, ws, bp, gs, L.ACT_NONE, dt)
        else:
            sc = xp
        h1 = _conv_fwd_raw(x, w0, None, g0, L.ACT_LRELU, dt)
        keep = any(ctx.needs_input_grad[:6])
        pool_ok = want_pool and res_pool_ok(h1, g2)
        bits_mode = keep and not _second_order() and "no_sign_bits" not in _DEBUG_DISPATCH
        r = _conv_fwd_raw(h1, w2, None, g2, L.ACT_LRELU, dt, res=sc, alpha=al, want2=keep and not bits_mode, want_sign=bits_mode,
                          want_pool=pool_ok, round_act=True)
        r = r if isinstance(r, tuple) else (r,)
        out = r[0]
        res = r[1] if keep else None
        outp = r[-1] if pool_ok else None
        ctx.geoms = (g0, g2, gs)
        ctx.learned = ws is not None
        ctx.has_bs = bs is not None
        ctx.save_for_backward(x, xp if ws is not None else None, h1, res, w0, w2, ws, gamma)
        if want_pool:
            if outp is None:
                outp = torch.empty((N, out.shape[1] // 2, out.shape[2] // 2, out.shape[3]), dtype=dt, device=x.device)
                L.call("xmc_sumpool2", _p(out), _p(outp), N, out.shape[1], out.shape[2], out.shape[3], 0.25, _code(dt), _st())
            ctx.mark_non_differentiable(outp)
            ctx.set_materialize_grads(False)
            return out, outp
        return out

    @staticmethod
    def backward(ctx, dout, _doutp=None):
        if dout is None:
            return (None,) * 11
        x, xp, h1, res, w0, w2, ws, gamma = ctx.saved_tensors
        need = tuple(bool(v) for v in ctx.needs_input_grad[:6])
        if res is not None and res.dtype == torch.uint8 and torch.is_grad_enabled():
            raise RuntimeError("ResDFn: this block kept only the sign bits of its residual branch; wrap the forward in "
                               "ops.second_order() to differentiate its backward (the MA-GP pattern)")
        outs = ResDBwdFn.apply(dout, x, xp, h1, res, w0, w2, ws, gamma, ctx.geoms, ctx.learned, ctx.has_bs, need, _skip_wgrad())
        return tuple(outs) + (None, None, None, None, None)


def dstem_eligible(xin, c_img, c_sc, c_out):
    return (xin.is_cuda and xin.dtype != torch.float32 and xin.shape[3] == 8 and xin.shape[1] % 16 == 0 and xin.shape[2] % 64 == 0 and
            c_img == 32 and c_out == 64 and c_sc and "no_dstem" not in _DEBUG_DISPATCH)


class DStemBlockFn(torch.autograd.Function):

    @staticmethod
    def forward(ctx, xin, w_img, b_img, w0, w2, ws, bs, gamma, g_img, g0, g2, gs, want_pool=False):
        xin = xin.contiguous()
        dt = xin.dtype
        N, H, W, _ = xin.shape
        OH, OW = H // 2, W // 2
        wsets, bias, D, DB = _dstem_compose_raw(w_img, b_img, w0, ws, bs)
        al = gamma.detach().reshape(-1).float()
        keep = any(ctx.needs_input_grad[:8])
        pool_ok = want_pool and H % 4 == 0 and W % 4 == 0
        so2 = _second_order()
        fuse_sc = pool_ok and OH % 8 == 0 and OW % 32 == 0 and not so2 and "no_scimg" not in _DEBUG_DISPATCH
        h1, sc = _dstem_fwd_raw(xin, wsets, bias, want_sc=not fuse_sc)
        _dstem_border_fwd_raw(xin, wsets, bias, D, DB, h1)
        assert pool_ok == (want_pool and res_pool_ok(h1, g2))
        r = None
        if fuse_sc:
            r = _conv_fwd_raw(h1, w2, None, g2, L.ACT_LRELU, dt, alpha=al, want_sign=keep, want_pool=pool_ok, round_act=True,
                              sc_img=_dstem_sc_operands(xin, wsets, bias))
            if r is None:
                _, sc = _dstem_fwd_raw(xin, wsets, bias, want_sc=True)
        if r is None:
            r = _conv_fwd_raw(h1, w2, None, g2, L.ACT_LRELU, dt, res=sc, alpha=al, want_sign=keep and not so2, want2=keep and so2,
                              want_pool=pool_ok, round_act=True)
        r = r if isinstance(r, tuple) else (r,)
        out = r[0]
        bits = r[1] if keep else None
        outp = r[-1] if pool_ok else None
        ctx.geoms = (g_img, g0, g2, gs)
        ctx.has_bs = bs is not None
        ctx.save_for_backward(xin, h1, bits, w_img, b_img, w0, w2, ws, bs, gamma, wsets, D)
        if want_pool:
            if outp is None:
                outp = torch.empty((N, out.shape[1] // 2, out.shape[2] // 2, out.shape[3]), dtype=dt, device=xin.device)
                L.call("xmc_sumpool2", _p(out), _p(outp), N, out.shape[1], out.shape[2], out.shape[3], 0.25, _code(dt), _st())
            ctx.mark_non_differentiable(outp)
            ctx.set_materialize_grads(False)
            return out, outp
        return out

    @staticmethod
    def backward(ctx, dout, _doutp=None):
        nin = 13
        if dout is None:
            return (None,) * nin
        xin, h1, bits, w_img, b_img, w0, w2, ws, bs, gamma, wsets, D = ctx.saved_tensors
        if bits is not None and bits.dtype != torch.uint8:
            need = tuple(bool(v) for v in ctx.needs_input_grad[:8])
            outs = DStemBwdFn.apply(dout, xin, h1, bits, w_img, b_img, w0, w2, ws, bs, gamma, ctx.geoms, need, _skip_wgrad())
            return tuple(outs) + (None,) * 5
        if torch.is_grad_enabled():
            raise RuntimeError("DStemBlockFn: this block kept only the sign bits of its residual branch; wrap the forward in "
                               "ops.second_order() to differentiate its backward (the MA-GP pattern)")
        with torch.no_grad():
            return DStemBlockFn._backward_bits(ctx, dout)

    @staticmethod
    def _backward_bits(ctx, dout):
        nin = 13
        xin, h1, bits, w_img, b_img, w0, w2, ws, bs, gamma, wsets, D = ctx.saved_tensors
        g_img, g0, g2, gs = ctx.geoms
# ... 125 lines not shown
            if learned and need[0] and "no_pw1x1_masked_src" not in _DEBUG_DISPATCH:
                dxp_early, gr = _conv_dgrad_raw(dout, ws, gs, (xp.shape[1], xp.shape[2]), dt, src_bits=res)
            if gr is None:
                gr = torch.empty_like(dout)
                L.call("xmc_signmask_apply", _p(dout), _p(res), _p(gr), dout.numel(), 0.2, _code(dt), _st())
            dw2 = _conv_wgrad_raw(h1, gr, g2, scale=al).view(w2.shape) if (need[2] and not skip_w) else None
            gh = _conv_dgrad_raw(gr, w2, g2, (h1.shape[1], h1.shape[2]), dt, mask=h1, alpha=al, dot=dgam)
        else:
            dxp_early = None
            gr = torch.empty_like(res)
            L.call("xmc_scale_mask_dot", _p(dout), _p(res), _p(al), _p(gr), _p(dgam), res.numel(), _code(dt), _st())
            dw2 = _conv_wgrad_raw(h1, gr, g2).view(w2.shape) if (need[2] and not skip_w) else None
            gh = _conv_dgrad_raw(gr, w2, g2, (h1.shape[1], h1.shape[2]), dt, mask=h1)
        dw0 = _conv_wgrad_raw(x, gh, g0).view(w0.shape) if (need[1] and not skip_w) else None
        dws = dbs = None
        if learned:
            if need[3] and not skip_w:
                if has_bs and need[4]:
                    dws, dbs = _conv_wgrad_raw(xp, dout, gs, want_bias=True)
                    dbs = dbs[: gs.cout]
                else:
                    dws = _conv_wgrad_raw(xp, dout, gs)
                dws = dws.view(ws.shape)
            dxp = dxp_early if dxp_early is not None else (_conv_dgrad_raw(dout, ws, gs, (xp.shape[1], xp.shape[2]), dt) if need[0] else None)
        else:
            dxp = dout
        dx = None
        if need[0]:
            dx = _conv_dgrad_raw(gh, w0, g0, (x.shape[1], x.shape[2]), dt, res=dxp, res_rows=True, res_scale=0.25)
        dgamma = dgam.reshape(gamma.shape).to(gamma.dtype) if need[5] else None
        ctx.geoms, ctx.learned = geoms, learned
        ctx.save_for_backward(dout, h1, res, w0, w2, ws, gamma, gr, gh)
        return dx, dw0, dw2, dws, dbs, dgamma

    @staticmethod
    @torch.autograd.function.once_differentiable
    def backward(ctx, g, g_dw0=None, g_dw2=None, g_dws=None, g_dbs=None, g_dgamma=None):
        if any(t is not None for t in (g_dw0, g_dw2, g_dws, g_dbs, g_dgamma)):
            raise NotImplementedError("ResDBwdFn: only d(dx) is differentiated again (the MA-GP penalty); use ops.composable() "
                                      "for second derivatives through the weight gradients")
        nin = 14
        if g is None:
            return (None,) * nin
        dout, h1, res, w0, w2, ws, gamma, gr, gh = ctx.saved_tensors
        g0, g2, gs = ctx.geoms
        dt = h1.dtype
        g = g.contiguous()
        if g.dtype != dt:
            g = g.to(dt)
        N, H, W, Cx = g.shape
        skip_w = _skip_wgrad()
        al = gamma.detach().reshape(-1).float()
        gp = torch.empty((N, H // 2, W // 2, Cx), dtype=dt, device=g.device)
        L.call("xmc_sumpool2", _p(g), _p(gp), N, H, W, Cx, 0.25, _code(dt), _st())
        sc = _conv_fwd_raw(gp, ws, None, gs, L.ACT_NONE, dt) if ctx.learned else gp
        v = _conv_fwd_raw(g, w0, None, g0, L.ACT_NONE, dt, mask=h1)
        ddout, c2 = _conv_fwd_raw(v, w2, None, g2, L.ACT_NONE, dt, res=sc, alpha=al, mask=res, want2=True)
        dgamma = None
        if ctx.needs_input_grad[8]:
            u = torch.empty_like(c2)
            L.call("xmc_lrelu_mask", _p(c2), _p(res), _p(u), c2.numel(), 0.2, _code(dt), _st())
            dg = _zeros_f32_out(1, g.device)
            L.call("xmc_dot", _p(dout), _p(u), _p(dg), u.numel(), _code(dt), _st())
            dgamma = dg.reshape(gamma.shape).to(gamma.dtype)
        dw0 = dw2 = dws = None
        if not skip_w:
            if ctx.needs_input_grad[5]:
                dw0 = _conv_wgrad_raw(g, gh, g0).view(w0.shape)
            if ctx.needs_input_grad[6]:
                dw2 = _conv_wgrad_raw(v, gr, g2).view(w2.shape)
            if ctx.learned and ctx.needs_input_grad[7]:
                dws = _conv_wgrad_raw(gp, dout, gs).view(ws.shape)
        return (ddout.to(ctx.dout_dtype) if ctx.needs_input_grad[0] else None, None, None, None, None, dw0, dw2, dws, dgamma,
                None, None, None, None, None)


def res_pool_ok(h1, g2):
    OH, OW = g2.out_hw(h1.shape[1], h1.shape[2])
    return OH % 2 == 0 and OW % 2 == 0


class Affine2LreluFn(torch.autograd.Function):

    @staticmethod
    def forward(ctx, x, g0, b0, g1, b1, slope=0.2):
        x = x.contiguous()
        two = g1 is not None
        ps = [t.contiguous().float() for t in ((g0, b0, g1, b1) if two else (g0, b0))]
        y = _affine_fwd_raw(x, ps, slope)
        ctx.two, ctx.slope = two, float(slope)
        ctx.save_for_backward(x, *ps)
        return y

    @staticmethod
    @torch.autograd.function.once_differentiable
    def backward(ctx, dy):
        x, *ps = ctx.saved_tensors
        dx, red = _affine_bwd_raw(x, dy.contiguous(), ps, ctx.slope)
        if ctx.two:
            return dx, red[0], red[1], red[2], red[3], None
        return dx, red[0], red[1], None, None, None


def _gn_fwd_raw(x, wf, bf, groups, slope, eps):
    N, H, W, Cc = x.shape
    y = torch.empty_like(x)
    stats = torch.empty((N, groups, 2), dtype=torch.float32, device=x.device)
    ws = _zeros_f32((N, Cc, 2), x.device)
    L.call("xmc_groupnorm_fwd", _p(x), _p(wf), _p(bf), _p(y), _p(stats), _p(ws), N, H * W, Cc, groups, float(eps),
           float(slope), _code(x.dtype), _st())
    return y, stats


def _gn_bwd_raw(x, dy, wf, bf, stats, groups, slope):
    N, H, W, Cc = x.shape
    dx = torch.empty_like(x)
    dw, db = torch.empty_like(wf), torch.empty_like(bf)
    ws = _zeros_f32(N * Cc * 2 + N * groups * 2, x.device)
    L.call("xmc_groupnorm_bwd", _p(x), _p(dy), _p(wf), _p(bf), _p(stats), _p(dx), _p(dw), _p(db), _p(ws), N, H * W, Cc,
           groups, float(slope), _code(x.dtype), _st())
    return dx, dw, db


class Affine2LreluSkipFn(torch.autograd.Function):

    @staticmethod
    def forward(ctx, x, g0, b0, g1, b1, pool_grad=False):
        x = x.contiguous()
        ps = [t.contiguous().float() for t in (g0, b0, g1, b1)]
        y = _affine_fwd_raw(x, ps, 0.2)
        ctx.set_materialize_grads(False)
        ctx.pool = bool(pool_grad)
        ctx.save_for_backward(x, *ps)
        return y, x.view_as(x)

    @staticmethod
    @torch.autograd.function.once_differentiable
    def backward(ctx, dy, dskip):
        x, *ps = ctx.saved_tensors
        if dy is None:
            return dskip, None, None, None, None, None
        if ctx.pool and x.shape[1] % 2 == 0 and x.shape[2] % 2 == 0 and x.shape[3] // 8 in (1, 2, 4, 8, 16, 32):
            dx, red, dxp = _affine_bwd_raw(x, dy.contiguous(), ps, 0.2, dx_acc=dskip, want_sumpool=True)
            _pooled_put(dx, dxp)
        else:
            dx, red = _affine_bwd_raw(x, dy.contiguous(), ps, 0.2, dx_acc=dskip)
        return dx, red[0], red[1], red[2], red[3], None


def affine2_lrelu_skip(x, g0, b0, g1, b1, pool_grad=False):
    return Affine2LreluSkipFn.apply(x, g0, b0, g1, b1, pool_grad)


class GroupNormFn(torch.autograd.Function):

    @staticmethod
    def forward(ctx, x, w, b, groups, slope, eps):
        x = x.contiguous()
        wf, bf = w.detach().float().contiguous(), b.detach().float().contiguous()
        y, stats = _gn_fwd_raw(x, wf, bf, groups, slope, eps)
        ctx.groups, ctx.slope = groups, slope
        ctx.save_for_backward(x, wf, bf, stats)
        return y

    @staticmethod
    @torch.autograd.function.once_differentiable
    def backward(ctx, dy):
        x, wf, bf, stats = ctx.saved_tensors
        dx, dw, db = _gn_bwd_raw(x, dy.contiguous(), wf, bf, stats, ctx.groups, ctx.slope)
        return dx, dw, db, None, None, None


class BatchNormTrainFn(torch.autograd.Function):

    @staticmethod
    def forward(ctx, x, w, b, eps):
        x = x.contiguous()
        N, H, W, Cc = x.shape
        wf, bf = w.detach().float().contiguous(), b.detach().float().contiguous()
        y = torch.empty_like(x)
        stats = torch.empty((1, Cc, 2), dtype=torch.float32, device=x.device)
        ws = _zeros_f32((1, Cc, 2), x.device)
        L.call("xmc_groupnorm_fwd", _p(x), _p(wf), _p(bf), _p(y), _p(stats), _p(ws), 1, N * H * W, Cc, Cc, float(eps), -1.0,
               _code(x.dtype), _st())
        ctx.save_for_backward(x, wf, bf, stats)
        out_stats = stats.view(Cc, 2)
        ctx.mark_non_differentiable(out_stats)
        return y, out_stats

    @staticmethod
    @torch.autograd.function.once_differentiable
    def backward(ctx, dy, _dstats):
        x, wf, bf, stats = ctx.saved_tensors
        dy = dy.contiguous()
        N, H, W, Cc = x.shape
        dx = torch.empty_like(x)
        dw, db = torch.empty_like(wf), torch.empty_like(bf)
        ws = _zeros_f32(Cc * 2 + Cc * 2, x.device)
        L.call("xmc_groupnorm_bwd", _p(x), _p(dy), _p(wf), _p(bf), _p(stats), _p(dx), _p(dw), _p(db), _p(ws), 1, N * H * W, Cc,
               Cc, -1.0, _code(x.dtype), _st())
        return dx, dw, db, None


def batchnorm_train(x, w, b, eps=1e-5):
    return BatchNormTrainFn.apply(x, w, b, eps)


def _attn_fwd_raw(key, q, x, ncon, scale):
    N, H, W, CK = key.shape
    pk, px = CK // ncon, x.shape[3] // ncon
    stats = torch.empty((N, ncon, 2), dtype=torch.float32, device=x.device)
    out = torch.empty((N, ncon, px), dtype=torch.float32, device=x.device)
    ws = torch.empty(int(L.load().xmc_attn_pool_ws_floats(N, H * W)), dtype=torch.float32, device=x.device)
    L.call("xmc_attn_pool_fwd", _p(key), _p(q), _p(x), _p(stats), _p(out), _p(ws), N, H * W, ncon, pk, px, float(scale),
           _code(x.dtype), _st())
    return out, stats


def _attn_bwd_raw(key, q, x, stats, out, dctx, ncon, scale, dx_acc=None):
    N, H, W, CK = key.shape
    pk, px = CK // ncon, x.shape[3] // ncon
    dq = _zeros_f32_out(tuple(q.shape), q.device)
    dkey = torch.empty_like(key)
    dx = torch.empty_like(x) if dx_acc is None else dx_acc
    assert dx.shape == x.shape and dx.dtype == x.dtype and dx.is_contiguous()
    L.call("xmc_attn_pool_bwd_acc", _p(key), _p(q), _p(x), _p(stats), _p(out), _p(dctx), _p(dq), _p(dkey), _p(dx), _p(dx_acc),
           N, H * W, ncon, pk, px, float(scale), _code(x.dtype), _st())
    return dkey, dq, dx


class WordRegionPoolFn(torch.autograd.Function):

    @staticmethod
    def forward(ctx, qmap, kh, pad):
        qmap, kh = qmap.contiguous(), kh.contiguous().float()
        _need_cuda(qmap, kh)
        B, H, W, Cq = qmap.shape
        T = kh.shape[2]
        assert Cq == 64 and kh.shape == (B, 16, T, 4) and pad.shape == (B, T), (qmap.shape, kh.shape, pad.shape)
        padu = pad.to(torch.uint8).contiguous()
        out = _zeros_f32_out((B, 16, 4), qmap.device)
        L.call("xmc_word_pool_fwd", _p(qmap), _p(kh), _p(padu), _p(out), B, H * W, 16, 4, T, _code(qmap.dtype), _st())
        ctx.save_for_backward(qmap, kh, padu)
        return out

    @staticmethod
    @torch.autograd.function.once_differentiable
    def backward(ctx, dctx):
        qmap, kh, padu = ctx.saved_tensors
        B, H, W, _ = qmap.shape
        T = kh.shape[2]
        dq = torch.empty_like(qmap)
        dkh = _zeros_f32_out((B, 16, T, 4), qmap.device)
        L.call("xmc_word_pool_bwd", _p(qmap), _p(kh), _p(padu), _p(dctx.contiguous().float()), _p(dq), _p(dkh), B, H * W, 16, 4, T,
               _code(qmap.dtype), _st())
        return dq, dkh, None


def word_region_pool(qmap, kh, pad):
    return WordRegionPoolFn.apply(qmap, kh, pad)


class AttnPoolFn(torch.autograd.Function):

    @staticmethod
    def forward(ctx, key, q, x, ncon, scale):
        key, x = key.contiguous(), x.contiguous()
        q = q.contiguous().float()
        out, stats = _attn_fwd_raw(key, q, x, ncon, scale)
        ctx.ncon, ctx.scale = ncon, scale
        ctx.save_for_backward(key, q, x, stats, out)
        return out

    @staticmethod
    @torch.autograd.function.once_differentiable
    def backward(ctx, dctx):
        key, q, x, stats, out = ctx.saved_tensors
        dkey, dq, dx = _attn_bwd_raw(key, q, x, stats, out, dctx.contiguous().float(), ctx.ncon, ctx.scale)
        return dkey, dq, dx, None, None
```

### xmc_gan/model/df_gan.py

```python
from collections import OrderedDict

import torch
import torch.nn as nn

from xmc_gan_amd import ops
from xmc_gan_amd.lib import ACT_LRELU, ACT_NONE, ACT_RELU, ACT_TANH

from .modules import HipConv2d, HipLinear, as_nchw_view, as_nhwc, conv2d_nxn, linear


def gen_arch(img_size, nch):
    assert img_size in [64, 128, 256]
    depth = {64: 5, 128: 6, 256: 7}[img_size]
    mult = [8] * (depth - 2) + [4, 2, 1]
    return {
        'in_channels': [m * nch for m in mult[:-1]],
        'out_channels': [m * nch for m in mult[1:]],
        'upsample': [True] * (depth - 1) + [False],
        'resolution': [8 << i for i in range(depth - 1)] + [img_size],
        'depth': depth,
    }


def disc_arch(img_size, nch):
# ... 75 lines not shown
            out = ops.upsample2(out)
        return self.tail(out, lrelu_done, return_nhwc, nhwc_dst)


class NetD(nn.Module):
    def __init__(self, cfg, **kwargs):
        super(NetD, self).__init__()
        ndf = cfg.TRAIN.NCH
        spec_norm = cfg.DISC.SPEC_NORM
        arch = disc_arch(img_size=cfg.IMG.SIZE, nch=ndf)
        self.conv_img = conv2d_nxn(in_dim=arch['in_channels'][0], out_dim=arch['out_channels'][0], kernel_size=3,
                                   stride=1, padding=1, spec_norm=spec_norm)
        self.downblocks = nn.ModuleList(
            [resD(in_dim=arch['in_channels'][i], out_dim=arch['out_channels'][i],
                  downsample=arch['downsample'][i], spec_norm=spec_norm) for i in range(1, arch['depth'])])
        self.COND_DNET = D_GET_LOGITS(cfg, ndf=ndf, spec_norm=spec_norm)

    def forward(self, x, nhwc8=None, **kwargs):
        pooled = None
        xin = ops.to_nhwc8(x) if nhwc8 is None else nhwc8
        src = x if nhwc8 is None else nhwc8
        leaf_in = torch.is_tensor(src) and src.requires_grad and src.is_leaf
        with ops.second_order(leaf_in or ops.second_order_active()):
            nblk = len(self.downblocks)
            b0 = self.downblocks[0]
            first = 0
            sink, cut = self.cut_sink, self.cut_block()
            if (ops.fused_blocks() and not self.conv_img.spec_norm and b0.downsample
                    and not (ops.second_order_active() and ops.debug_switch("no_dstem2"))
                    and ops.dstem_eligible(xin, self.conv_img.out_channels, b0.learned_shortcut, b0.conv_r[0].out_channels)):
                r0, r2, s_ = b0.conv_r[0], b0.conv_r[2], b0.conv_s
                out, pooled = ops.DStemBlockFn.apply(xin, self.conv_img.weight, self.conv_img.bias, r0.weight, r2.weight, s_.weight, s_.bias,
                                                     b0.gamma, self.conv_img.geom, r0.geom, r2.geom, s_.geom, nblk > 1)
                first = 1
            elif ops.fused_blocks() and xin.is_cuda and xin.shape[1] % 2 == 0:
                out, pooled = self.conv_img(xin, want_pool=True)
            else:
                out = self.conv_img(xin)
            for i, block in enumerate(self.downblocks):
                if i < first:
                    if sink is not None and i == cut:
                        sink.extend(t for t in (out, pooled) if torch.is_tensor(t) and t.requires_grad)
                    continue
                out, pooled = block(out, xp_hint=pooled, want_pool=i + 1 < nblk)
                if sink is not None and i == cut:
                    sink.extend(t for t in (out, pooled) if torch.is_tensor(t) and t.requires_grad)
        return as_nchw_view(out)

    cut_sink = None

    def cut_block(self):
        k = len(self.downblocks) - 4
        return k if k >= 0 and not self.conv_img.spec_norm else None

    def late_parameters(self):
        k = self.cut_block()
        early = list(self.conv_img.parameters()) + [p for b in self.downblocks[:k + 1] for p in b.parameters()]
        ids = {id(p) for p in early}
        return [p for p in self.parameters() if id(p) not in ids], early


class D_GET_LOGITS(nn.Module):

    def __init__(self, cfg, ndf, spec_norm=False):
        super(D_GET_LOGITS, self).__init__()
        nef = cfg.TRAIN.NEF
        text_dim = cfg.TEXT.EMBEDDING_DIM
        self.img_match = cfg.DISC.IMG_MATCH
        if self.img_match:
            self.proj_match = linear(ndf * 16, nef, spec_norm=spec_norm)
            cond_dim = nef
        elif cfg.DISC.SENT_MATCH:
            self.proj_match = linear(nef, ndf * 16, spec_norm=spec_norm)
            cond_dim = ndf * 16
        elif cfg.DISC.SEPERATE and (text_dim != nef):
            self.proj_match = linear(text_dim, nef, spec_norm=spec_norm)
            cond_dim = nef
        else:
            self.proj_match = nn.Identity()
            cond_dim = text_dim
        self.joint_conv = nn.Sequential(
            conv2d_nxn(in_dim=ndf * 16 + cond_dim, out_dim=ndf * 2, kernel_size=3, stride=1, padding=1, bias=False,
                       spec_norm=spec_norm),
            nn.LeakyReLU(0.2, inplace=True),
            conv2d_nxn(in_dim=ndf * 2, out_dim=1, kernel_size=4, stride=1, padding=0, bias=False, spec_norm=spec_norm),
        )

    def forward(self, x, sent_embs, **kwargs):
        xh = as_nhwc(x)
        B = xh.size(0)
        out = ops.global_avgpool(xh)
        sent_embs = sent_embs.float()
        if self.img_match:
            out = self.proj_match(out)
        else:
            sent_embs = self.proj_match(sent_embs)
        c = ops.cast(_pad8(sent_embs), xh.dtype)
        c = c.view(B, 1, 1, -1).expand(B, xh.size(1), xh.size(2), c.size(-1))
        h_c_code = torch.cat((xh, c), 3)
        j0 = self.joint_conv[0]
        if h_c_code.dtype == torch.float32 and ops.act_dtype() != torch.float32 and not j0.spec_norm and j0.bias is None:
            m = ops.pair_conv2d(h_c_code, j0.weight, j0.geom, ACT_LRELU)
        else:
            m = j0(h_c_code, act=ACT_LRELU)
        m = self.joint_conv[2](m, out_dtype=torch.float32)
        match = as_nchw_view(m[..., :1])
        return [match, out, sent_embs]


def _pad8(t):
    r = (-t.size(-1)) % 8
    return t if r == 0 else torch.nn.functional.pad(t, (0, r))


class G_Block(nn.Module):
    def __init__(self, in_dim, out_dim, cond_dim, upsample):
        super(G_Block, self).__init__()
        self.learnable_sc = (in_dim != out_dim)
        self.upsample = upsample
        self.c1 = HipConv2d(in_dim, out_dim, 3, 1, 1)
        self.c2 = HipConv2d(out_dim, out_dim, 3, 1, 1)
        self.affine0 = affine(num_features=in_dim, cond_dim=cond_dim)
        self.affine1 = affine(num_features=in_dim, cond_dim=cond_dim)
        self.affine2 = affine(num_features=out_dim, cond_dim=cond_dim)
        self.affine3 = affine(num_features=out_dim, cond_dim=cond_dim)
        self.gamma = nn.Parameter(torch.zeros(1))
        if self.learnable_sc:
            self.c_sc = HipConv2d(in_dim, out_dim, 1, stride=1, padding=0)

    def modulation_mlps(self):
        out = []
        for a in (self.affine0, self.affine1, self.affine2, self.affine3):
            for m in (a.fc_gamma, a.fc_beta):
                out.append((m.linear1.weight, m.linear1.bias, m.linear2.weight, m.linear2.bias))
        return out

    def modulation(self, c):
        return (*self.affine0.scale_shift(c), *self.affine1.scale_shift(c),
                *self.affine2.scale_shift(c), *self.affine3.scale_shift(c))

    def forward(self, x, c, mod=None):
        out = ops.axpby(self.shortcut(x), self.residual(x, c, mod), self.gamma)
        if self.upsample:
            out = ops.upsample2(out)
        return out

    def fuses_end(self, x, x_pending_up):
        return bool(x_pending_up) and ops.fused_blocks() and x.is_cuda

    def forward_fused(self, x, mod, x_pending_up, out_lrelu=False, tail=None, nhwc_dst=None, x_from_end=False):
        if not x_pending_up:
            out = ops.axpby(self.shortcut(x), self.residual(x, None, mod), self.gamma)
            return ops.lrelu(out) if out_lrelu else out
        h, xs = ops.affine2_lrelu_skip(x, *mod[0:4], pool_grad=x_from_end) if x.is_cuda else (ops.affine2_lrelu(x, *mod[0:4]), x)
        h = ops.upconv3x3(h, self.c1.weight, self.c1.bias, self.c1.geom)
        if self.fuses_end(x, x_pending_up) and (tail is not None or not out_lrelu):
            return ops.g_block_end(h, mod[4:8], self.c2.weight, self.c2.bias, self.c2.geom, self.shortcut(xs), self.gamma,
                                   tail=tail, nhwc_dst=nhwc_dst)
        assert tail is None
        h = ops.affine2_lrelu(h, *mod[4:8])
        if not out_lrelu and ops.fused_blocks() and h.shape[1] % 2 == 0:
            return ops.conv_axpby_up(h, self.c2.weight, self.c2.bias, self.c2.geom, self.shortcut(xs), self.gamma)
        return ops.axpby_up(self.shortcut(xs), self.c2(h), self.gamma, lrelu=out_lrelu)

    def shortcut(self, x):
        return self.c_sc(x, pair=ops.precise_trunk()) if self.learnable_sc else x

    def residual(self, x, c, mod=None):
        m = self.modulation(c) if mod is None else mod
        h = ops.affine2_lrelu(x, *m[0:4])
        h = self.c1(h)
        h = ops.affine2_lrelu(h, *m[4:8])
        return self.c2(h)


class _CondMLP(nn.Module):

    def __init__(self, cond_dim, num_features):
        super().__init__()
        self.linear1 = HipLinear(cond_dim, 256)
        self.relu1 = nn.ReLU(inplace=True)
        self.linear2 = HipLinear(256, num_features)

    def forward(self, y):
        return self.linear2(self.linear1(y, act=ACT_RELU))


class affine(nn.Module):
    def __init__(self, num_features, cond_dim):
        super(affine, self).__init__()
        self.fc_gamma = _CondMLP(cond_dim, num_features)
        self.fc_beta = _CondMLP(cond_dim, num_features)
        self._initialize()

    def _initialize(self):
        nn.init.zeros_(self.fc_gamma.linear2.weight.data)
        nn.init.ones_(self.fc_gamma.linear2.bias.data)
        nn.init.zeros_(self.fc_beta.linear2.weight.data)
        nn.init.zeros_(self.fc_beta.linear2.bias.data)

    def scale_shift(self, y):
        return self.fc_gamma(y), self.fc_beta(y)

    def forward(self, x, y=None):
        w, b = self.scale_shift(y)
        return x * w[:, None, None, :].to(x.dtype) + b[:, None, None, :].to(x.dtype)


class resD(nn.Module):
    def __init__(self, in_dim, out_dim, downsample, spec_norm=False):
        super().__init__()
        self.downsample = downsample
        self.learned_shortcut = (in_dim != out_dim)
        self.conv_r = nn.Sequential(
            conv2d_nxn(in_dim=in_dim, out_dim=out_dim, kernel_size=4, stride=2, padding=1, bias=False, spec_norm=spec_norm),
            nn.LeakyReLU(0.2, inplace=True),
            conv2d_nxn(in_dim=out_dim, out_dim=out_dim, kernel_size=3, stride=1, padding=1, bias=False, spec_norm=spec_norm),
            nn.LeakyReLU(0.2, inplace=True),
        )
        self.conv_s = conv2d_nxn(in_dim=in_dim, out_dim=out_dim, kernel_size=1, stride=1, padding=0, spec_norm=spec_norm)
        self.gamma = nn.Parameter(torch.zeros(1))

    def forward(self, x, c=None, xp_hint=None, want_pool=None):
        if self.downsample and ops.fused_blocks() and x.is_cuda:
            r0, r2, s_ = self.conv_r[0], self.conv_r[2], self.conv_s
            r = ops.ResDFn.apply(x, r0.effective_weight(), r2.effective_weight(),
                                 s_.effective_weight() if self.learned_shortcut else None,
                                 s_.bias if self.learned_shortcut else None, self.gamma, r0.geom, r2.geom, s_.geom,
                                 xp_hint, bool(want_pool))
            if want_pool is None:
                return r
            return r if want_pool else (r, None)
        out = ops.axpby(self.shortcut(x), self.residual(x), self.gamma)
        return out if want_pool is None else (out, None)

    def shortcut(self, x):
        if self.downsample:
            x = ops.avgpool2(x)
        if self.learned_shortcut:
            x = self.conv_s(x)
        return x

    def residual(self, x):
        r = self.conv_r[0](x, act=ACT_LRELU)
        return self.conv_r[2](r, act=ACT_LRELU)
```

Measured before the change: 6062 images/s.

## Fuse generator block entry affine pair with 1x1 shortcut conv in one pass

Adds fused forward and backward kernels for the generator block entry. The forward applies the two affine+LeakyReLU modulations and computes the learnable 1x1 shortcut conv from a single read of x. The backward fuses the shortcut dgrad with the affine-pair backward and optional sum-pool of dx. The goal is fewer kernel launches and fewer passes over large NHWC activations in the late, high-resolution blocks. It adds per-sample parameter staging, atomics for the modulation-gradient reductions and a more complex dispatch, and falls back to the old path for unsupported shapes.

```diff
diff --git a/include/xmc_gan_hip.h b/include/xmc_gan_hip.h
--- a/include/xmc_gan_hip.h
+++ b/include/xmc_gan_hip.h
@@ -114,6 +114,11 @@
 int xmc_conv_ptile_scimg(const XmcConvDesc* d, void* stream);
 int xmc_conv_wgrad_bits(const XmcConvDesc* d, float* dwp, void* stream);
 int xmc_gtail_bwd(const XmcConvDesc* d, const void* img, float* dwp, float* dbias, int dw_rows, int grid_cap, void* stream);
+int xmc_gentry_fwd(const void* x, const float* g0, const float* b0, const float* g1, const float* b1, const void* wpk, const float* bias,
+                   void* h, void* sc, int N, int H, int W, int Cin, int Cout, int wrows, float slope, int dtype, int grid_cap, void* stream);
+int xmc_gentry_bwd(const void* x, const void* dy, const void* dsc, const float* g0, const float* b0, const float* g1, const float* b1,
+                   const void* wpk_t, void* dx, void* dx_pool, float* dg0, float* db0, float* dg1, float* db1, int N, int H, int W,
+                   int Cin, int Cout, int wrows, float slope, int dtype, int grid_cap, void* stream);
 int xmc_tanh_bwd(const void* dy, const void* y, void* dx, int64_t n, int dtype, void* stream);
 int xmc_axpby(const void* a, const void* b, const float* alpha_dev, void* y, int64_t n, int dtype, void* stream);
 int xmc_axpby_up(const void* a, const void* b, const float* alpha_dev, void* y, int N, int H, int W, int C, int dtype, void* stream);
diff --git a/xmc-gan_amd/csrc/common.h b/xmc-gan_amd/csrc/common.h
--- a/xmc-gan_amd/csrc/common.h
+++ b/xmc-gan_amd/csrc/common.h
@@ -65,6 +65,37 @@
 }
 __device__ __forceinline__ float lrelu_slope(float ref) { return ref > 0.f ? 1.f : XMC_LRELU; }
 __device__ __forceinline__ float tanh_bwd_f(float dy, float y) { return xmc_pin_f32(dy * (1.f - y * y)); }
+__device__ __forceinline__ float affine2_fwd_f(float x, float g0, float b0, float g1, float b1, float slope, bool two) {
+    float u = __builtin_fmaf(x, g0, b0);
+    u = u > 0.f ? u : slope * u;
+    const float t = __builtin_fmaf(u, g1, b1);
+    return xmc_pin_f32(two ? (t > 0.f ? t : slope * t) : u);
+}
+template <int DT>
+__device__ __forceinline__ void affine2_bwd_unit(float (&xv)[8], const float (&dv)[8], const float (&o)[8], bool has_in, bool two, float slope,
+                                                 float al, float* dacc, const float (&G0)[8], const float (&B0)[8], const float (&G1)[8],
+                                                 const float (&B1)[8], float (&sg0)[8], float (&sb0)[8], float (&sg1)[8], float (&sb1)[8]) {
+#pragma unroll
+    for (int k = 0; k < 8; ++k) {
+        const float u = __builtin_fmaf(xv[k], G0[k], B0[k]);
+        const float a1 = u > 0.f ? u : slope * u;
+        const float v = __builtin_fmaf(a1, G1[k], B1[k]);
+        if (dacc) {
+            const float y2 = two ? (v > 0.f ? v : slope * v) : a1;
+            *dacc += dv[k] * (DT == XMC_BF16 ? (float)(xmc_h16)y2 : y2);
+        }
+        const float dvk = dv[k] * al;
+        const float dvv = two ? dvk * (v > 0.f ? 1.f : slope) : dvk;
+        sg1[k] += dvv * a1; sb1[k] += dvv;
+        const float du = dvv * G1[k] * (u > 0.f ? 1.f : slope);
+        sg0[k] += du * xv[k]; sb0[k] += du;
+        xv[k] = xmc_pin_f32(du * G0[k]);
+    }
+    if (has_in) {
+#pragma unroll
+        for (int k = 0; k < 8; ++k) xv[k] += o[k];
+    }
+}
 __device__ __forceinline__ u32x4 xmc_apply_sign_bits(u32x4 v, unsigned b) {
     bf16x8 h = __builtin_bit_cast(bf16x8, v);
 #pragma unroll
diff --git a/xmc-gan_amd/csrc/conv_thin.hip b/xmc-gan_amd/csrc/conv_thin.hip
--- a/xmc-gan_amd/csrc/conv_thin.hip
+++ b/xmc-gan_amd/csrc/conv_thin.hip
@@ -569,6 +569,360 @@
         hipLaunchKernelGGL((pw1x1w_kernel<KS, false>), dim3(nb, ny), dim3(512), lds, st, d, ngroups, ncols, nullptr, nullptr, 0.f);
     }
     xmc_note_kernel(smasked ? "pw1x1w_kernel<%d, true>" : "pw1x1w_kernel<%d>", KS);
+    XMC_LAUNCH_CHECK();
+    return 0;
+}
+
+struct GEntryArgs {
+    const void *x, *dy, *dsc, *wpk;
+    void *h, *sc, *dx, *dx_pool;
+    const float *bias, *g0, *b0, *g1, *b1;
+    float *dg0, *db0, *dg1, *db1;
+    int N, H, W, gpi, nvg, per;
+    float slope;
+};
+
+template <int KS, int TN, bool WLDS, int NW>
+__device__ __forceinline__ void gentry_weights(const u32x4* __restrict__ w16, unsigned char* wlds, u32x4 (&wf)[WLDS ? 1 : KS][WLDS ? 1 : TN], int tid, int fr, int fc) {
+    constexpr int RSTR = KS * 64 + 16;
+    if constexpr (WLDS) {
+        for (int id = tid; id < TN * 16 * KS * 4; id += NW * 64) {
+            const int row = id / (KS * 4), ch = id - row * (KS * 4);
+            const int j = row >> 4, r = row & 15;
+            const int lrow = (j >> 1) * 32 + (r >> 2) * 8 + (j & 1) * 4 + (r & 3);
+            *reinterpret_cast<u32x4*>(wlds + row * RSTR + ch * 16) = w16[(size_t)lrow * (KS * 4) + ch];
+        }
+        __syncthreads();
+    } else {
+#pragma unroll
+        for (int j = 0; j < TN; ++j) {
+            const int lrow = (j >> 1) * 32 + (fr >> 2) * 8 + (j & 1) * 4 + (fr & 3);
+#pragma unroll
+            for (int ks = 0; ks < KS; ++ks) wf[ks][j] = w16[(size_t)lrow * (KS * 4) + ks * 4 + fc];
+        }
+    }
+}
+
+template <int KS, int TN, bool WLDS, int NW>
+__global__ __launch_bounds__(NW * 64) void gentry_fwd_kernel(const GEntryArgs a) {
+    extern __shared__ __attribute__((aligned(16))) unsigned char glds[];
+    constexpr int CIN = KS * 32, C8 = KS * 4, CO8 = TN * 2, UNR = 4;
+    constexpr int RSTR = KS * 64 + 16, WBYTES = WLDS ? TN * 16 * RSTR : 0;
+    const int tid = threadIdx.x, lane = tid & 63, wv = tid >> 6, fr = lane & 15, fc = lane >> 4;
+    const u32x4* __restrict__ src16 = reinterpret_cast<const u32x4*>(a.x);
+    bf16x8* __restrict__ h8 = reinterpret_cast<bf16x8*>(a.h);
+    bf16x8* __restrict__ sc8 = reinterpret_cast<bf16x8*>(a.sc);
+    float* const par = reinterpret_cast<float*>(glds + WBYTES) + wv * 4 * CIN;
+    u32x4 wf[WLDS ? 1 : KS][WLDS ? 1 : TN];
+    gentry_weights<KS, TN, WLDS, NW>(reinterpret_cast<const u32x4*>(a.wpk), glds, wf, tid, fr, fc);
+    float bias8[WLDS ? 1 : TN / 2][8];
+    if constexpr (!WLDS) {
+#pragma unroll
+        for (int u = 0; u < TN / 2; ++u)
+#pragma unroll
+            for (int c = 0; c < 8; ++c) bias8[u][c] = a.bias ? a.bias[u * 32 + fc * 8 + c] : 0.f;
+    }
+    const float slope = a.slope, one = 1.f;
+    const int HW = a.H * a.W;
+    const int lo = blockIdx.x * a.per, hi = min(lo + a.per, a.nvg);
+    int cur = -1;
+    for (int g0 = lo + wv * UNR; g0 < hi; g0 += NW * UNR) {
+        const int n = g0 / a.gpi, gl0 = g0 - n * a.gpi;
+        if (n != cur) {
+            const float* vec[4] = {a.g0, a.b0, a.g1, a.b1};
+            __builtin_amdgcn_wave_barrier();
+#pragma unroll
+            for (int q = 0; q < 4; ++q)
+                for (int c = lane; c < CIN; c += 64) par[q * CIN + c] = vec[q][(size_t)n * CIN + c];
+            __builtin_amdgcn_wave_barrier();
+            cur = n;
+        }
+        size_t pix[UNR];
+        bool ok[UNR];
+        u32x4 pf[UNR][KS];
+#pragma unroll
+        for (int r = 0; r < UNR; ++r) {
+            const int p = (gl0 + r) * 16 + fr;
+            ok[r] = p < HW;
+            pix[r] = (size_t)n * HW + (ok[r] ? p : HW - 1);
+#pragma unroll
+            for (int ks = 0; ks < KS; ++ks) pf[r][ks] = src16[pix[r] * C8 + ks * 4 + fc];
+        }
+#pragma unroll
+        for (int ks = 0; ks < KS; ++ks) {
+            const f32x4* pq = reinterpret_cast<const f32x4*>(par + (ks * 4 + fc) * 8);
+            float P[4][8];
+#pragma unroll
+            for (int q = 0; q < 4; ++q) {
+                const f32x4 lo4 = pq[q * (CIN / 4)], hi4 = pq[q * (CIN / 4) + 1];
+#pragma unroll
+                for (int k = 0; k < 4; ++k) { P[q][k] = lo4[k]; P[q][4 + k] = hi4[k]; }
+            }
+#pragma unroll
+            for (int r = 0; r < UNR; ++r) {
+                const bf16x8 xv = __builtin_bit_cast(bf16x8, pf[r][ks]);
+                bf16x8 o;
+#pragma unroll
+                for (int k = 0; k < 8; ++k) o[k] = (xmc_h16)affine2_fwd_f((float)xv[k], P[0][k], P[1][k], P[2][k], P[3][k], slope, true);
+                if (ok[r]) h8[pix[r] * C8 + ks * 4 + fc] = o;
+            }
+        }
+        if constexpr (!WLDS) {
+#pragma unroll
+            for (int r = 0; r < UNR; ++r) {
+                if ((gl0 + r) * 16 >= HW) break;
+                f32x4 acc[TN];
+#pragma unroll
+                for (int j = 0; j < TN; ++j) acc[j] = f32x4{0.f, 0.f, 0.f, 0.f};
+#pragma unroll
+                for (int ks = 0; ks < KS; ++ks)
+#pragma unroll
+                    for (int j = 0; j < TN; ++j)
+                        acc[j] = XMC_MFMA_16x16x32(__builtin_bit_cast(bf16x8, wf[ks][j]), __builtin_bit_cast(bf16x8, pf[r][ks]), acc[j], 0, 0, 0);
+#pragma unroll
+                for (int u = 0; u < TN / 2; ++u) {
+                    bf16x8 o;
+#pragma unroll
+                    for (int q = 0; q < 4; ++q) {
+                        const float x0 = acc[2 * u][q] + bias8[u][q], x1 = acc[2 * u + 1][q] + bias8[u][4 + q];
+                        o[q] = (xmc_h16)fmaxf(x0, x0 * one);
+                        o[4 + q] = (xmc_h16)fmaxf(x1, x1 * one);
+                    }
+                    if (ok[r]) sc8[pix[r] * CO8 + u * 4 + fc] = o;
+                }
+            }
+        } else {
+#pragma unroll 1
+            for (int u = 0; u < TN / 2; ++u) {
+                f32x4 acc[UNR][2];
+#pragma unroll
+                for (int r = 0; r < UNR; ++r) acc[r][0] = acc[r][1] = f32x4{0.f, 0.f, 0.f, 0.f};
+                const unsigned char* const wr = glds + (u * 32 + fr) * RSTR + fc * 16;
+#pragma unroll
+                for (int ks = 0; ks < KS; ++ks) {
+                    const bf16x8 wa = *reinterpret_cast<const bf16x8*>(wr + ks * 64), wb = *reinterpret_cast<const bf16x8*>(wr + 16 * RSTR + ks * 64);
+#pragma unroll
+                    for (int r = 0; r < UNR; ++r) {
+                        acc[r][0] = XMC_MFMA_16x16x32(wa, __builtin_bit_cast(bf16x8, pf[r][ks]), acc[r][0], 0, 0, 0);
+                        acc[r][1] = XMC_MFMA_16x16x32(wb, __builtin_bit_cast(bf16x8, pf[r][ks]), acc[r][1], 0, 0, 0);
+                    }
+                }
+                float b8[8];
+#pragma unroll
+                for (int c = 0; c < 8; ++c) b8[c] = a.bias ? a.bias[u * 32 + fc * 8 + c] : 0.f;
+#pragma unroll
+                for (int r = 0; r < UNR; ++r) {
+                    bf16x8 o;
+#pragma unroll
+                    for (int q = 0; q < 4; ++q) {
+                        const float x0 = acc[r][0][q] + b8[q], x1 = acc[r][1][q] + b8[4 + q];
+                        o[q] = (xmc_h16)fmaxf(x0, x0 * one);
+                        o[4 + q] = (xmc_h16)fmaxf(x1, x1 * one);
+                    }
+                    if (ok[r]) sc8[pix[r] * CO8 + u * 4 + fc] = o;
+                }
+            }
+        }
+    }
+}
+
+template <int KS, int TN, bool WLDS, bool POOL, int NW>
+__global__ __launch_bounds__(NW * 64, NW == 4 ? 2 : 1) void gentry_bwd_kernel(const GEntryArgs a) {
+    extern __shared__ __attribute__((aligned(16))) unsigned char glds[];
+    constexpr int C8 = TN * 2, CS8 = KS * 4, PPS = 64 / C8, NPAIR = C8 / 8;
+    constexpr int RSTR = KS * 64 + 16, WBYTES = WLDS ? TN * 16 * RSTR : 0, SSTR = C8 * 16 + 16;
+    const int tid = threadIdx.x, lane = tid & 63, wv = tid >> 6, fr = lane & 15, fc = lane >> 4;
+    const int cc = lane % C8, pg = lane / C8;
+    const u32x4* __restrict__ x16 = reinterpret_cast<const u32x4*>(a.x);
+    const u32x4* __restrict__ dy16 = reinterpret_cast<const u32x4*>(a.dy);
+    const u32x4* __restrict__ dsc16 = reinterpret_cast<const u32x4*>(a.dsc);
+    unsigned char* const slab = glds + WBYTES + wv * 16 * SSTR;
+    u32x4 wf[WLDS ? 1 : KS][WLDS ? 1 : TN];
+    gentry_weights<KS, TN, WLDS, NW>(reinterpret_cast<const u32x4*>(a.wpk), glds, wf, tid, fr, fc);
+    const float slope = a.slope;
+    const int HW = a.H * a.W, Wq = a.W >> 1;
+    const int nunits = POOL ? (a.H >> 1) * Wq : HW;
+    auto slot_pixel = [&](int gl, int f) -> int {
+        if constexpr (POOL) {
+            const int s = f / PPS, pl = f % PPS;
+            const int q = gl * 4 + (s >> 1) * (PPS / 2) + (pl >> 1);
+            if (q >= nunits) return -1;
+            const int qy = q / Wq, qx = q - qy * Wq;
+            return (2 * qy + (s & 1)) * a.W + 2 * qx + (pl & 1);
+        } else {
+            const int p = gl * 16 + f;
+            return p < nunits ? p : -1;
+        }
+    };
+    float G0[8], B0[8], G1[8], B1[8], sg0[8], sb0[8], sg1[8], sb1[8];
+#pragma unroll
+    for (int k = 0; k < 8; ++k) sg0[k] = sb0[k] = sg1[k] = sb1[k] = 0.f;
+    auto flush = [&](int n) {
+        float* const outs[4] = {a.dg0, a.db0, a.dg1, a.db1};
+        float* const sums[4] = {sg0, sb0, sg1, sb1};
+#pragma unroll
+        for (int q = 0; q < 4; ++q)
+#pragma unroll
+            for (int k = 0; k < 8; ++k) {
+                float v = sums[q][k];
+#pragma unroll
+                for (int o = C8; o < 64; o <<= 1) v += __shfl_xor(v, o, 64);
+                if (lane < C8) atomicAdd(&outs[q][((size_t)n * C8 + cc) * 8 + k], v);
+                sums[q][k] = 0.f;
+            }
+    };
+    auto load_dsc = [&](int g, u32x4 (&pf)[KS]) {
+        const int n = g / a.gpi, p = slot_pixel(g - n * a.gpi, fr);
+        const size_t idx = ((size_t)n * HW + (p < 0 ? 0 : p)) * CS8;
+#pragma unroll
+        for (int ks = 0; ks < KS; ++ks) pf[ks] = dsc16[idx + ks * 4 + fc];
+    };
+    struct PairOps { int px[2]; u32x4 xq[2], dq[2]; };
+    auto load_pair = [&](int g, int t, PairOps& o) {
+        const int n = g / a.gpi, gl = g - n * a.gpi;
+#pragma unroll
+        for (int e = 0; e < 2; ++e) {
+            o.px[e] = slot_pixel(gl, (2 * t + e) * PPS + pg);
+            const size_t idx = ((size_t)n * HW + (o.px[e] < 0 ? 0 : o.px[e])) * C8 + cc;
+            o.xq[e] = x16[idx];
+            o.dq[e] = dy16[idx];
+        }
+    };
+    const int lo = blockIdx.x * a.per, hi = min(lo + a.per, a.nvg);
+    int g = lo + wv, cur = -1;
+    u32x4 pfs[KS];
+    PairOps cu;
+    constexpr bool PRE = KS < 4;
+    if (g < hi) { load_dsc(g, pfs); load_pair(g, 0, cu); }
+    for (; g < hi; g += NW) {
+        const int n = g / a.gpi, gl = g - n * a.gpi;
+        if (n != cur) {
+            if (cur >= 0) flush(cur);
+            const size_t pb = ((size_t)n * C8 + cc) * 8;
+#pragma unroll
+            for (int k = 0; k < 8; ++k) { G0[k] = a.g0[pb + k]; B0[k] = a.b0[pb + k]; G1[k] = a.g1[pb + k]; B1[k] = a.b1[pb + k]; }
+            cur = n;
+        }
+        u32x4 pfn[KS];
+        if (PRE && g + NW < hi) load_dsc(g + NW, pfn);
+        else {
+#pragma unroll
+            for (int ks = 0; ks < KS; ++ks) pfn[ks] = pfs[ks];
+        }
+#pragma unroll
+        for (int u = 0; u < TN / 2; ++u) {
+            f32x4 acc0 = {0.f, 0.f, 0.f, 0.f}, acc1 = {0.f, 0.f, 0.f, 0.f};
+#pragma unroll
+            for (int ks = 0; ks < KS; ++ks) {
+                bf16x8 wa, wb;
+                if constexpr (WLDS) {
+                    const unsigned char* const wr = glds + (u * 32 + fr) * RSTR + fc * 16 + ks * 64;
+                    wa = *reinterpret_cast<const bf16x8*>(wr);
+                    wb = *reinterpret_cast<const bf16x8*>(wr + 16 * RSTR);
+                } else {
+                    wa = __builtin_bit_cast(bf16x8, wf[ks][2 * u]);
+                    wb = __builtin_bit_cast(bf16x8, wf[ks][2 * u + 1]);
+                }
+                acc0 = XMC_MFMA_16x16x32(wa, __builtin_bit_cast(bf16x8, pfs[ks]), acc0, 0, 0, 0);
+                acc1 = XMC_MFMA_16x16x32(wb, __builtin_bit_cast(bf16x8, pfs[ks]), acc1, 0, 0, 0);
+            }
+            bf16x8 o;
+#pragma unroll
+            for (int q = 0; q < 4; ++q) {
+                o[q] = (xmc_h16)(acc0[q] + 0.f);
+                o[4 + q] = (xmc_h16)(acc1[q] + 0.f);
+            }
+            *reinterpret_cast<bf16x8*>(slab + fr * SSTR + (u * 4 + fc) * 16) = o;
+        }
+        __builtin_amdgcn_wave_barrier();
+#pragma unroll 1
+        for (int t = 0; t < NPAIR; ++t) {
+            const bool more = t + 1 < NPAIR;
+            const int gn = more ? g : g + NW;
+            PairOps nx = cu;
+            if (gn < hi) load_pair(gn, more ? t + 1 : 0, nx);
+            float acc8[8] = {0, 0, 0, 0, 0, 0, 0, 0};
+#pragma unroll
+            for (int e = 0; e < 2; ++e) {
+                const bool live = cu.px[e] >= 0;
+                const bf16x8 xb = __builtin_bit_cast(bf16x8, cu.xq[e]), db = __builtin_bit_cast(bf16x8, cu.dq[e]);
+                const bf16x8 ob = *reinterpret_cast<const bf16x8*>(slab + ((2 * t + e) * PPS + pg) * SSTR + cc * 16);
+                float xv[8], dv[8], ov[8];
+#pragma unroll
+                for (int k = 0; k < 8; ++k) { xv[k] = (float)xb[k]; dv[k] = live ? (float)db[k] : 0.f; ov[k] = live ? (float)ob[k] : 0.f; }
+                affine2_bwd_unit<XMC_BF16>(xv, dv, ov, true, true, slope, 1.f, nullptr, G0, B0, G1, B1, sg0, sb0, sg1, sb1);
+                if (live) Vec8<XMC_BF16>::store(a.dx, ((size_t)n * HW + cu.px[e]) * C8 + cc, xv);
+                if (POOL) {
+#pragma unroll
+                    for (int k = 0; k < 8; ++k) acc8[k] += (float)(xmc_h16)xv[k];
+                }
+                __builtin_amdgcn_sched_barrier(0);
+            }
+            if (POOL) {
+#pragma unroll
+                for (int k = 0; k < 8; ++k) acc8[k] += __shfl_xor(acc8[k], C8, 64);
+                const int q = gl * 4 + t * (PPS / 2) + (pg >> 1);
+                if ((pg & 1) == 0 && cu.px[0] >= 0) Vec8<XMC_BF16>::store(a.dx_pool, ((size_t)n * nunits + q) * C8 + cc, acc8);
+            }
+            cu = nx;
+        }
+        __builtin_amdgcn_wave_barrier();
+        if (PRE) {
+#pragma unroll
+            for (int ks = 0; ks < KS; ++ks) pfs[ks] = pfn[ks];
+        } else if (g + NW < hi) {
+            load_dsc(g + NW, pfs);
+        }
+    }
+    if (cur >= 0) flush(cur);
+}
+
+template <typename K>
+int gentry_resident(K kernel, int threads, size_t lds) {
+    int dev = 0, cus = 0, nb = 0;
+    if (hipGetDevice(&dev) != hipSuccess || hipDeviceGetAttribute(&cus, hipDeviceAttributeMultiprocessorCount, dev) != hipSuccess || cus < 1) cus = 256;
+    if (hipOccupancyMaxActiveBlocksPerMultiprocessor(&nb, kernel, threads, lds) != hipSuccess || nb < 1) nb = 1;
+    (void)hipGetLastError();
+    return cus * nb;
+}
+
+inline int gentry_grid(GEntryArgs& a, int resident, int grid_cap, int unit) {
+    int gx = resident;
+    if (grid_cap > 0 && gx > grid_cap) gx = grid_cap;
+    const int chunks = (a.nvg + unit - 1) / unit;
+    if (gx > chunks) gx = chunks;
+    a.per = (chunks + gx - 1) / gx * unit;
+    return (a.nvg + a.per - 1) / a.per;
+}
+
+template <int KS, int TN, bool WLDS, int NW>
+int launch_gentry_fwd(GEntryArgs& a, int grid_cap, hipStream_t st) {
+    constexpr size_t lds = (WLDS ? TN * 16 * (KS * 64 + 16) : 0) + NW * 4 * KS * 32 * sizeof(float);
+    auto kernel = gentry_fwd_kernel<KS, TN, WLDS, NW>;
+    if (lds > 64 * 1024) XMC_ALLOW_BIG_LDS((*kernel));
+    static const int resident = gentry_resident(kernel, NW * 64, lds);
+    const int gx = gentry_grid(a, resident, grid_cap, 4);
+    hipLaunchKernelGGL(kernel, dim3(gx), dim3(NW * 64), lds, st, a);
+    xmc_note_kernel("gentry_fwd_kernel<%d, %d>", KS, TN);
+    XMC_LAUNCH_CHECK();
+    return 0;
+}
+
+template <int KS, int TN, bool WLDS, int NW>
+int launch_gentry_bwd(GEntryArgs& a, int grid_cap, hipStream_t st) {
+    constexpr size_t lds = (WLDS ? TN * 16 * (KS * 64 + 16) : 0) + NW * 16 * (TN * 2 * 16 + 16);
+    if (a.dx_pool) {
+        auto kernel = gentry_bwd_kernel<KS, TN, WLDS, true, NW>;
+        if (lds > 64 * 1024) XMC_ALLOW_BIG_LDS((*kernel));
+        static const int resident = gentry_resident(kernel, NW * 64, lds);
+        hipLaunchKernelGGL(kernel, dim3(gentry_grid(a, resident, grid_cap, 1)), dim3(NW * 64), lds, st, a);
+    } else {
+        auto kernel = gentry_bwd_kernel<KS, TN, WLDS, false, NW>;
+        if (lds > 64 * 1024) XMC_ALLOW_BIG_LDS((*kernel));
+        static const int resident = gentry_resident(kernel, NW * 64, lds);
+        hipLaunchKernelGGL(kernel, dim3(gentry_grid(a, resident, grid_cap, 1)), dim3(NW * 64), lds, st, a);
+    }
+    xmc_note_kernel("gentry_bwd_kernel<%d, %d, %d>", KS, TN, a.dx_pool ? 1 : 0);
     XMC_LAUNCH_CHECK();
     return 0;
 }
@@ -741,6 +1095,53 @@
     return 0;
 }
 
+static int gentry_case(int N, int H, int W, int Cin, int Cout, int dtype) {
+    static const bool off = xmc_debug_off("no_gentry_fused");
+    if (off || dtype != XMC_BF16) return 1;
+    if (!((Cin == 64 && Cout == 32) || (Cin == 128 && Cout == 64) || (Cin == 256 && Cout == 128))) return 1;
+    if ((int64_t)N * H * W * (Cin / 8) >= (1ll << 31) || (int64_t)N * ((int64_t)H * W / 16 + 4) >= (1ll << 30)) return 1;
+    return 0;
+}
+
+extern "C" int xmc_gentry_fwd(const void* x, const float* g0, const float* b0, const float* g1, const float* b1, const void* wpk, const float* bias,
+                              void* h, void* sc, int N, int H, int W, int Cin, int Cout, int wrows, float slope, int dtype, int grid_cap, void* stream) {
+    if (!x || !g0 || !b0 || !g1 || !b1 || !wpk || !h || !sc) return XMC_EINVAL;
+    if (N < 1 || H < 1 || W < 1 || Cin < 8 || Cout < 8 || Cin % 8 || Cout % 8) return XMC_ESHAPE;
+    if (const int rc = gentry_case(N, H, W, Cin, Cout, dtype)) return rc;
+    if (wrows != Cout) return 1;
+    GEntryArgs a = {};
+    a.x = x; a.wpk = wpk; a.h = h; a.sc = sc; a.bias = bias;
+    a.g0 = g0; a.b0 = b0; a.g1 = g1; a.b1 = b1;
+    a.N = N; a.H = H; a.W = W; a.slope = slope;
+    a.gpi = ((H * W + 15) / 16 + 3) / 4 * 4;
+    a.nvg = N * a.gpi;
+    hipStream_t st = reinterpret_cast<hipStream_t>(stream);
+    if (Cin == 64) return launch_gentry_fwd<2, 2, false, 4>(a, grid_cap, st);
+    if (Cin == 128) return launch_gentry_fwd<4, 4, true, 4>(a, grid_cap, st);
+    return launch_gentry_fwd<8, 8, true, 8>(a, grid_cap, st);
+}
+
+extern "C" int xmc_gentry_bwd(const void* x, const void* dy, const void* dsc, const float* g0, const float* b0, const float* g1, const float* b1,
+                              const void* wpk_t, void* dx, void* dx_pool, float* dg0, float* db0, float* dg1, float* db1, int N, int H, int W,
+                              int Cin, int Cout, int wrows, float slope, int dtype, int grid_cap, void* stream) {
+    if (!x || !dy || !dsc || !g0 || !b0 || !g1 || !b1 || !wpk_t || !dx || !dg0 || !db0 || !dg1 || !db1) return XMC_EINVAL;
+    if (N < 1 || H < 1 || W < 1 || Cin < 8 || Cout < 8 || Cin % 8 || Cout % 8) return XMC_ESHAPE;
+    if (const int rc = gentry_case(N, H, W, Cin, Cout, dtype)) return rc;
+    if (wrows != Cin) return 1;
+    if (dx_pool && ((H & 1) || (W & 1))) return 1;
+    GEntryArgs a = {};
+    a.x = x; a.dy = dy; a.dsc = dsc; a.wpk = wpk_t; a.dx = dx; a.dx_pool = dx_pool;
+    a.g0 = g0; a.b0 = b0; a.g1 = g1; a.b1 = b1;
+    a.dg0 = dg0; a.db0 = db0; a.dg1 = dg1; a.db1 = db1;
+    a.N = N; a.H = H; a.W = W; a.slope = slope;
+    a.gpi = dx_pool ? ((H / 2) * (W / 2) + 3) / 4 : (H * W + 15) / 16;
+    a.nvg = N * a.gpi;
+    hipStream_t st = reinterpret_cast<hipStream_t>(stream);
+    if (Cin == 64) return launch_gentry_bwd<1, 4, false, 4>(a, grid_cap, st);
+    if (Cin == 128) return launch_gentry_bwd<2, 8, true, 4>(a, grid_cap, st);
+    return launch_gentry_bwd<4, 16, true, 8>(a, grid_cap, st);
+}
+
 static int pw1x1_go(const XmcConvDesc* d, void* stream, const unsigned char* sbits, void* smasked, float mslope) {
     static const bool off = xmc_debug_off("no_pw1x1");
     if (off) return 1;
diff --git a/xmc-gan_amd/csrc/pointwise.hip b/xmc-gan_amd/csrc/pointwise.hip
--- a/xmc-gan_amd/csrc/pointwise.hip
+++ b/xmc-gan_amd/csrc/pointwise.hip
@@ -351,12 +351,7 @@
         const size_t idx = ((size_t)n * HW + p) * C8 + cc;
         Vec8<DT>::load(x, idx, v);
 #pragma unroll
-        for (int k = 0; k < 8; ++k) {
-            float u = v[k] * G0[k] + B0[k];
-            u = u > 0.f ? u : slope * u;
-            const float t = u * G1[k] + B1[k];
-            v[k] = two ? (t > 0.f ? t : slope * t) : u;
-        }
+        for (int k = 0; k < 8; ++k) v[k] = affine2_fwd_f(v[k], G0[k], B0[k], G1[k], B1[k], slope, two);
         Vec8<DT>::store(y, idx, v);
     }
 }
@@ -380,26 +375,7 @@
         sg0[k] = sb0[k] = sg1[k] = sb1[k] = 0.f;
     }
     auto pixel = [&](size_t idx, float (&xv)[8], const float (&dv)[8], const float (&o)[8], float* acc8) {
-#pragma unroll
-        for (int k = 0; k < 8; ++k) {
-            float u = xv[k] * G0[k] + B0[k];
-            float a1 = u > 0.f ? u : slope * u;
-            float v = a1 * G1[k] + B1[k];
-            if (dot) {
-                const float y2 = two ? (v > 0.f ? v : slope * v) : a1;
-                dacc += dv[k] * (DT == XMC_BF16 ? (float)(xmc_h16)y2 : y2);
-            }
-            const float dvk = dv[k] * al;
-            float dvv = two ? dvk * (v > 0.f ? 1.f : slope) : dvk;
-            sg1[k] += dvv * a1; sb1[k] += dvv;
-            float du = dvv * G1[k] * (u > 0.f ? 1.f : slope);
-            sg0[k] += du * xv[k]; sb0[k] += du;
-            xv[k] = du * G0[k];
-        }
-        if (dx_in) {
-#pragma unroll
-            for (int k = 0; k < 8; ++k) xv[k] += o[k];
-        }
+        affine2_bwd_unit<DT>(xv, dv, o, dx_in != nullptr, two, slope, al, dot ? &dacc : nullptr, G0, B0, G1, B1, sg0, sb0, sg1, sb1);
         Vec8<DT>::store(dx, idx, xv);
         if (POOL) {
 #pragma unroll
diff --git a/xmc-gan_amd/lib.py b/xmc-gan_amd/lib.py
--- a/xmc-gan_amd/lib.py
+++ b/xmc-gan_amd/lib.py
@@ -80,6 +80,8 @@
     "xmc_conv_ptile_scimg": [C.POINTER(ConvDesc), vp],
     "xmc_conv_wgrad_bits": [C.POINTER(ConvDesc), vp, vp],
     "xmc_gtail_bwd": [C.POINTER(ConvDesc), vp, vp, vp, i32, i32, vp],
+    "xmc_gentry_fwd": [vp, vp, vp, vp, vp, vp, vp, vp, vp, i32, i32, i32, i32, i32, i32, f32, i32, i32, vp],
+    "xmc_gentry_bwd": [vp, vp, vp, vp, vp, vp, vp, vp, vp, vp, vp, vp, vp, vp, i32, i32, i32, i32, i32, i32, f32, i32, i32, vp],
     "xmc_tanh_bwd": [vp, vp, vp, i64, i32, vp],
     "xmc_axpby": [vp, vp, vp, vp, i64, i32, vp],
     "xmc_scale_mask_dot": [vp, vp, vp, vp, vp, i64, i32, vp],
diff --git a/xmc-gan_amd/ops/_engine.py b/xmc-gan_amd/ops/_engine.py
--- a/xmc-gan_amd/ops/_engine.py
+++ b/xmc-gan_amd/ops/_engine.py
@@ -684,6 +684,54 @@
     return (dx, red, dxp) if want_sumpool else (dx, red)
 
 
+def _gentry_accepts(x, geom, pair=False):
+    return (x.is_cuda and x.dim() == 4 and x.dtype != torch.float32 and not pair and "no_gentry_fused" not in _DEBUG_DISPATCH
+            and geom.k == 1 and geom.s == 1 and geom.p == 0 and geom.groups == 1 and geom.row_perm is None
+            and geom.cin == x.shape[3] and (geom.cin, geom.cout) in ((64, 32), (128, 64), (256, 128)))
+
+
+def _gentry_fwd_raw(x, ps, w, bias, geom, pair=False, grid_cap=0):
+    if not _gentry_accepts(x, geom, pair):
+        return None
+    _need_cuda(x, w)
+    N, H, W, Cc = x.shape
+    for t in ps:
+        assert t.shape == (N, Cc) and t.dtype == torch.float32 and t.is_contiguous(), (t.shape, (N, Cc))
+    assert x.is_contiguous() and len(ps) == 4
+    wpk = _packed_cached(w, geom, 0, x.dtype)
+    h = torch.empty_like(x)
+    sc = torch.empty((N, H, W, geom.cout), dtype=x.dtype, device=x.device)
+    with prof.launch("gentry_fwd_kernel (affine pair + 1x1 shortcut, one pass)", 2.0 * N * H * W * geom.cout * geom.cin,
+                     f"gentry-fwd {x.dtype} N{N} {H}x{W} {geom.cin}->{geom.cout}", _nbytes(x, h, sc)):
+        rc = L.load().xmc_gentry_fwd(_p(x), *[_p(t) for t in ps], _p(wpk), _p(bias), _p(h), _p(sc), N, H, W, Cc, geom.cout,
+                                     wpk.shape[1], 0.2, _code(x.dtype), int(grid_cap), _st())
+    if rc == 1:
+        return None
+    L.check(rc, "xmc_gentry_fwd")
+    return h, sc
+
+
+def _gentry_bwd_raw(x, dy, dsc, ps, w, geom, want_sumpool=False, grid_cap=0):
+    N, H, W, Cc = x.shape
+    if not _gentry_accepts(x, geom) or (want_sumpool and (H % 2 or W % 2)):
+        return None
+    _need_cuda(x, dy, dsc, w)
+    assert dy.shape == x.shape and dy.dtype == x.dtype and dy.is_contiguous() and x.is_contiguous()
+    assert dsc.shape == (N, H, W, geom.cout) and dsc.dtype == x.dtype and dsc.is_contiguous() and len(ps) == 4
+    wpk = _packed_cached(w, geom, 1, x.dtype)
+    dx = torch.empty_like(x)
+    dxp = torch.empty((N, H // 2, W // 2, Cc), dtype=x.dtype, device=x.device) if want_sumpool else None
+    red = _zeros_f32((4, N, Cc), x.device)
+    with prof.launch("gentry_bwd_kernel (1x1 shortcut dgrad + affine pair backward, one pass)", 2.0 * N * H * W * geom.cout * geom.cin,
+                     f"gentry-bwd {x.dtype} N{N} {H}x{W} {geom.cin}->{geom.cout}", _nbytes(x, dy, dsc, dx, dxp)):
+        rc = L.load().xmc_gentry_bwd(_p(x), _p(dy), _p(dsc), *[_p(t) for t in ps], _p(wpk), _p(dx), _p(dxp), *[_p(red[i]) for i in range(4)],
+                                     N, H, W, Cc, geom.cout, wpk.shape[1], 0.2, _code(x.dtype), int(grid_cap), _st())
+    if rc == 1:
+        return None
+    L.check(rc, "xmc_gentry_bwd")
+    return dx, red, dxp
+
+
 def compose_dstem(w_img, b_img, w0, ws, bs):
     F = torch.nn.functional
     co, mid = w0.shape[0], w0.shape[1]
diff --git a/xmc-gan_amd/ops/_nodes_block.py b/xmc-gan_amd/ops/_nodes_block.py
--- a/xmc-gan_amd/ops/_nodes_block.py
+++ b/xmc-gan_amd/ops/_nodes_block.py
@@ -4,8 +4,8 @@
 from ._engine import (
     _StagedMask, _affine_bwd_raw, _affine_fwd_raw, _conv1x1_pair_raw, _conv_dgrad_raw, _conv_fwd_raw, _conv_wgrad_raw,
     _dstem_border_fwd_raw, _dstem_compose_bwd_raw, _dstem_compose_raw, _dstem_dgrad_raw, _dstem_fwd_raw, _dstem_sc_operands,
-    _dstem_wgrad_raw, _pooled_put, _zeros_f32, _zeros_f32_out)
-from ._nodes_leaf import CastFn
+    _dstem_wgrad_raw, _gentry_accepts, _gentry_bwd_raw, _gentry_fwd_raw, _pooled_put, _zeros_f32, _zeros_f32_out)
+from ._nodes_leaf import CastFn, ColSumFn
 from ._nodes_conv import _bias_padded
 
 
@@ -437,6 +437,64 @@
     return Affine2LreluSkipFn.apply(x, g0, b0, g1, b1, pool_grad)
 
 
+class GBlockEntryFn(torch.autograd.Function):
+
+    @staticmethod
+    def forward(ctx, x, g0, b0, g1, b1, w, b, geom, pool_grad=False):
+        x = x.contiguous()
+        ps = [t.contiguous().float() for t in (g0, b0, g1, b1)]
+        r = _gentry_fwd_raw(x, ps, w, _bias_padded(b, geom), geom)
+        if r is None:
+            raise RuntimeError("GBlockEntryFn: not a case of xmc_gentry_fwd (ask ops.g_block_entry, which returns None for those)")
+        ctx.set_materialize_grads(False)
+        ctx.geom, ctx.pool, ctx.has_b = geom, bool(pool_grad), b is not None
+        ctx.save_for_backward(x, w, *ps)
+        return r
+
+    @staticmethod
+    @torch.autograd.function.once_differentiable
+    def backward(ctx, dy, dsc):
+        x, w, *ps = ctx.saved_tensors
+        geom = ctx.geom
+        if dy is None and dsc is None:
+            return (None,) * 9
+        if dsc is not None:
+            dsc = dsc.contiguous()
+        dx, red = None, (None,) * 4
+        if dy is None:
+            if ctx.needs_input_grad[0]:
+                dx = _conv_dgrad_raw(dsc, w, geom, (x.shape[1], x.shape[2]), x.dtype)
+        else:
+            dy = dy.contiguous()
+            pool = ctx.pool and x.shape[1] % 2 == 0 and x.shape[2] % 2 == 0
+            r = _gentry_bwd_raw(x, dy, dsc, ps, w, geom, want_sumpool=pool) if dsc is not None else None
+            if r is None:
+                dskip = _conv_dgrad_raw(dsc, w, geom, (x.shape[1], x.shape[2]), x.dtype) if dsc is not None else None
+                r = _affine_bwd_raw(x, dy, ps, 0.2, dx_acc=dskip, want_sumpool=pool)
+                r = r if pool else (*r, None)
+            dx, red, dxp = r
+            if pool:
+                _pooled_put(dx, dxp)
+        dw = db = None
+        if dsc is not None and not _skip_wgrad():
+            want_b = ctx.has_b and ctx.needs_input_grad[6]
+            if ctx.needs_input_grad[5]:
+                gw = _conv_wgrad_raw(x, dsc, geom, want_bias=want_b)
+                dw, db = gw if want_b else (gw, None)
+                dw = dw.view(w.shape)
+            elif want_b:
+                db = ColSumFn.apply(dsc)
+            if db is not None:
+                db = db[: geom.cout]
+        return dx, red[0], red[1], red[2], red[3], dw, db, None, None
+
+
+def g_block_entry(x, mod4, w, b, geom, pool_grad=False, pair=False):
+    if not _gentry_accepts(x, geom, pair):
+        return None
+    return GBlockEntryFn.apply(x, *mod4, w, b, geom, pool_grad)
+
+
 class GroupNormFn(torch.autograd.Function):
 
     @staticmethod
diff --git a/xmc_gan/model/df_gan.py b/xmc_gan/model/df_gan.py
--- a/xmc_gan/model/df_gan.py
+++ b/xmc_gan/model/df_gan.py
@@ -251,16 +251,24 @@
         if not x_pending_up:
             out = ops.axpby(self.shortcut(x), self.residual(x, None, mod), self.gamma)
             return ops.lrelu(out) if out_lrelu else out
-        h, xs = ops.affine2_lrelu_skip(x, *mod[0:4], pool_grad=x_from_end) if x.is_cuda else (ops.affine2_lrelu(x, *mod[0:4]), x)
+        entry = None
+        if self.learnable_sc and x.is_cuda and not self.c_sc.spec_norm:
+            entry = ops.g_block_entry(x, mod[0:4], self.c_sc.weight, self.c_sc.bias, self.c_sc.geom, x_from_end, pair=ops.precise_trunk())
+        if entry is not None:
+            h, sc = entry
+        else:
+            h, xs = ops.affine2_lrelu_skip(x, *mod[0:4], pool_grad=x_from_end) if x.is_cuda else (ops.affine2_lrelu(x, *mod[0:4]), x)
+            sc = None
+        shortcut = (lambda: self.shortcut(xs)) if sc is None else (lambda: sc)
         h = ops.upconv3x3(h, self.c1.weight, self.c1.bias, self.c1.geom)
         if self.fuses_end(x, x_pending_up) and (tail is not None or not out_lrelu):
-            return ops.g_block_end(h, mod[4:8], self.c2.weight, self.c2.bias, self.c2.geom, self.shortcut(xs), self.gamma,
+            return ops.g_block_end(h, mod[4:8], self.c2.weight, self.c2.bias, self.c2.geom, shortcut(), self.gamma,
                                    tail=tail, nhwc_dst=nhwc_dst)
         assert tail is None
         h = ops.affine2_lrelu(h, *mod[4:8])
         if not out_lrelu and ops.fused_blocks() and h.shape[1] % 2 == 0:
-            return ops.conv_axpby_up(h, self.c2.weight, self.c2.bias, self.c2.geom, self.shortcut(xs), self.gamma)
-        return ops.axpby_up(self.shortcut(xs), self.c2(h), self.gamma, lrelu=out_lrelu)
+            return ops.conv_axpby_up(h, self.c2.weight, self.c2.bias, self.c2.geom, shortcut(), self.gamma)
+        return ops.axpby_up(shortcut(), self.c2(h), self.gamma, lrelu=out_lrelu)
 
     def shortcut(self, x):
         return self.c_sc(x, pair=ops.precise_trunk()) if self.learnable_sc else x
```

Measured after the change: 6124 images/s, median of 6. 1.01x the previous value.
